# t-taniai/LocalExpStereo

Hardware: AMD Instinct MI355X
Metric: Mcost-evals/s (pixels x hypotheses / s), guided-filter cost aggregation, 1500x1000x256 vol (higher is better)
Workload: dtype i32 fixed-point box sums (exact; i64 stage-2 window sums), f32 3x3 algebra and combination

## Files before the change

### localexpstereo_amd/csrc/les_hip_march.inc

```
int check_rects(const les_hip_ctx* c, const les_hip_rect& f, const les_hip_rect& t)
{
    if (f.w < 0 || f.h < 0 || t.w < 0 || t.h < 0) return fail(LES_HIP_ERR_ARG, "negative rect size");
    if (f.x < 0 || f.y < 0 || f.x + f.w > c->p.W || f.y + f.h > c->p.H) return fail(LES_HIP_ERR_ARG, "filterRect outside the image");
    if (t.w > 0 && t.h > 0 && (t.x < f.x || t.y < f.y || t.x + t.w > f.x + f.w || t.y + t.h > f.y + f.h))
        return fail(LES_HIP_ERR_ARG, "targetRect not inside filterRect");
    return LES_HIP_OK;
}

int build_jobs(const les_hip_ctx* c, int n, const les_hip_rect* frs, const les_hip_rect* trs, int out_slabs,
               std::vector<les::Job>& jobs)
{
    const int TW = c->strip->TW, R = c->R;
    const long long P = (long long)c->p.H * c->p.W;
    long long strips = 0;
    for (int i = 0; i < n; i++) {
        int rc = check_rects(c, frs[i], trs[i]);
        if (rc) return rc;
        if (trs[i].w > 0 && trs[i].h > 0) strips += (trs[i].w + TW - 1) / TW;
    }
    int max_rows = 1 << 30;
    if (strips > 0 && strips < 2048) {
        long long want = (2048 + strips - 1) / strips;
        int tallest = 0;
        for (int i = 0; i < n; i++) tallest = std::max(tallest, trs[i].h);
        max_rows = std::max<long long>(std::max(8 * R, 64), (tallest + want - 1) / want);
    }
    jobs.clear();
    for (int i = 0; i < n; i++) {
        const les_hip_rect &f = frs[i], &t = trs[i];
        if (t.w <= 0 || t.h <= 0) continue;
        for (int sy = 0; sy < t.h; sy += max_rows)
            for (int sx = 0; sx < t.w; sx += TW) {
                les::Job j;
                j.tx0 = t.x + sx; j.ty0 = t.y + sy;
                j.tw = std::min(TW, t.w - sx); j.th = std::min(max_rows, t.h - sy);
                j.cx0 = f.x; j.cy0 = f.y; j.cx1 = f.x + f.w; j.cy1 = f.y + f.h;
                j.out_off = (out_slabs ? (long long)(i / out_slabs) * P : 0) + (long long)j.ty0 * c->p.W + j.tx0;
                j.out_stride = c->p.W;
                j.plane_idx = i;
                jobs.push_back(j);
            }
    }
    std::stable_sort(jobs.begin(), jobs.end(), [](const les::Job& a, const les::Job& b) {
        if (a.tx0 != b.tx0) return a.tx0 < b.tx0;
        if (a.ty0 != b.ty0) return a.ty0 < b.ty0;
        return a.plane_idx < b.plane_idx;
    });
    return LES_HIP_OK;
}

bool build_march_jobs(les_hip_ctx* c, int n, const les_hip_rect* frs, const les_hip_rect* trs, int out_slabs,
                      std::vector<les::Job>& jobs, bool& ok, const MarchEntry*& entry)
{
    jobs.clear();
    ok = false;
    entry = nullptr;
    if (!c->march) return true;
    const int R = c->R, W = c->p.W, H = c->p.H;
    const long long P = (long long)H * W;
    ok = true;
    for (int i = 0; i < n; i++) {
        const les_hip_rect &f = frs[i], &t = trs[i];
        if (t.w <= 0 || t.h <= 0) continue;
        if ((f.x > 0 && t.x - f.x < 2 * R) || (f.x + f.w < W && (f.x + f.w) - (t.x + t.w) < 2 * R) ||
            (f.y > 0 && t.y - f.y < 2 * R) || (f.y + f.h < H && (f.y + f.h) - (t.y + t.h) < 2 * R)) ok = false;
    }
    if (!ok) {
        note_fallback(c->fallback_seen, FB_GEOMETRY, "a target rectangle lies closer than 2 x radius = %d pixels to a filterRect border that is not an image border", 2 * R);
        return true;
    }
    const int ncu = c->ncu;
    const MarchEntry* cands[2] = {c->march, find_march(c->R, 0)};
    const MarchEntry* m = c->march;
    int max_rows = 1 << 30;
    {
        double best = 1e300;
        const int row_opts[] = {1 << 30, 1024, 512, 384, 256, 192, 128, 96, 64, 48, 32};
        for (int g = 0; g < 2; g++) {
            const MarchEntry* e = cands[g];
            if (!e || (g == 1 && e == cands[0])) continue;
            if (const char* w = getenv("LES_HIP_MARCH_WIDE")) if ((atoi(w) != 0) != (g == 0)) continue;
            for (int ro : row_opts) {
                long long njobs = 0;
                int rows = 0, useful = 0;
                for (int i = 0; i < n; i++) {
                    const les_hip_rect& t = trs[i];
                    if (t.w <= 0 || t.h <= 0) continue;
                    const int ns = (t.w + e->TW - 1) / e->TW;
                    const int nr = (t.h + ro - 1) / ro, sh = (t.h + nr - 1) / nr;
                    njobs += (long long)ns * nr;
                    rows = std::max(rows, sh);
                    useful = std::max(useful, (t.w + ns - 1) / ns);
                }
                if (njobs == 0) continue;
                const long long wgs = (njobs + e->NJ - 1) / e->NJ;
                const double ticks = (double)((rows + 4 * R + e->BY - 1) / e->BY + 3);
                const double cost = (double)((wgs + ncu - 1) / ncu) * ticks * (1.0 + 1e-3 * (double)wgs / ncu) + (ro == (1 << 30) ? 0.0 : 1e-6);
                if (cost < best) { best = cost; m = e; max_rows = ro; }
            }
        }
    }
    if (const char* e = getenv("LES_HIP_MARCH_ROWS")) max_rows = std::max(1, atoi(e));
    entry = m;
    const int TW = m->TW, NJ = m->NJ;
    for (int i = 0; i < n; i++) {
        const les_hip_rect &f = frs[i], &t = trs[i];
        if (t.w <= 0 || t.h <= 0) continue;
        const int ns = (t.w + TW - 1) / TW, sw = (t.w + ns - 1) / ns;
        const int nr = (t.h + max_rows - 1) / max_rows, sh = (t.h + nr - 1) / nr;
        for (int sy = 0; sy < t.h; sy += sh)
            for (int sx = 0; sx < t.w; sx += sw) {
                les::Job j;
                j.tx0 = t.x + sx; j.ty0 = t.y + sy;
                j.tw = std::min(sw, t.w - sx); j.th = std::min(sh, t.h - sy);
                j.cx0 = f.x; j.cy0 = f.y; j.cx1 = f.x + f.w; j.cy1 = f.y + f.h;
                j.out_off = (out_slabs ? (long long)(i / out_slabs) * P : 0) + (long long)j.ty0 * W + j.tx0;
                j.out_stride = W;
                j.plane_idx = i;
                jobs.push_back(j);
            }
    }
    std::stable_sort(jobs.begin(), jobs.end(), [](const les::Job& a, const les::Job& b) {
        if (a.tx0 != b.tx0) return a.tx0 < b.tx0;
        if (a.ty0 != b.ty0) return a.ty0 < b.ty0;
        return a.plane_idx < b.plane_idx;
    });
    while (!jobs.empty() && jobs.size() % NJ) {
        les::Job pad = jobs.back();
        pad.tw = 0; pad.th = 0;
        jobs.push_back(pad);
    }
    return true;
}

int ensure_planes(les_hip_ctx* c, size_t n)
{
    if (n <= c->planes_cap) return LES_HIP_OK;
    if (c->d_planes) HIPCHECK(hipFree(c->d_planes));
    c->d_planes = nullptr; c->planes_cap = 0;
    size_t cap = std::max<size_t>(n, 1024);
    HIPCHECK(hipMalloc((void**)&c->d_planes, cap * sizeof(float4)));
    c->planes_cap = cap;
    return LES_HIP_OK;
}

struct RawPatches { const les::RawCall* calls; const long long* off; float* raw; int n, chunks; };

les::View strip_view(const les_hip_ctx* c, int mode)
{
    les::View view{c->v[mode].vol, c->v[mode].stats, c->v[mode].ipk, c->v[mode].ipk10, nullptr, nullptr, mode ? -1.0f : 1.0f, c->th_color, c->th_grad};
    if (c->naive) { view.feat_self = c->v[mode].feat; view.feat_other = c->v[1 - mode].feat; }
    return view;
}

int launch_march(les_hip_ctx* c, const MarchEntry* m, int mode, const les::Job* d_mjobs, int ngroups, const float4* d_planes, float* d_out, int check,
                 hipStream_t stream, const RawPatches* rp = nullptr)
{
    if (ngroups <= 0) return LES_HIP_OK;
    les::MarchView mv = c->v[mode].mv;
    if (c->naive) {
        if (!rp || !rp->raw || !c->v[1 - mode].feat) return fail(LES_HIP_ERR_ARG, "view %d was not supplied at creation", mode);
        hipLaunchKernelGGL(les::les_naive_raw_kernel, dim3(rp->n, rp->chunks), dim3(256), 0, stream, c->geom, strip_view(c, mode), rp->calls, d_planes, rp->raw);
        mv.vol = rp->raw; mv.raw_off = rp->off;
    }
    hipLaunchKernelGGL(m->fn, dim3(ngroups), dim3(m->NT), 0, stream, c->geom, mv, d_mjobs, d_planes, d_out, ngroups, check);
    HIPCHECK(hipGetLastError());
    return LES_HIP_OK;
}

const StripEntry* strip_for(const les_hip_ctx* c) { return (c->naive || c->interp == 1) ? c->strip : c->istrip[c->interp == 0 ? 0 : 1]; }

int launch_strips(les_hip_ctx* c, int mode, const les::Job* d_jobs, int njobs, const float4* d_planes, float* d_out, int check, hipStream_t stream)
{
    if (njobs <= 0) return LES_HIP_OK;
    if (mode < 0 || mode > 1 || !c->v[mode].stats || (c->naive ? !c->v[1 - mode].feat : !c->v[mode].vol))
        return fail(LES_HIP_ERR_ARG, "view %d was not supplied at creation", mode);
    const StripEntry* se = strip_for(c);
    if (!se) return fail(LES_HIP_ERR_UNSUPPORTED, "no strip kernel for interpolation %d at guided-filter radius %d", c->interp, c->R);
    const les::View view = strip_view(c, mode);
    hipLaunchKernelGGL(se->fn, dim3(njobs), dim3(se->NT), 0, stream, c->geom, view, d_jobs, d_planes, d_out, njobs, check);
    HIPCHECK(hipGetLastError());
    return LES_HIP_OK;
}

bool interp_march_ok(const les_hip_ctx* c, int mode)
{
    return !c->naive && c->interp != 1 && c->march && c->v[mode].march_ok && (c->interp == 0 || c->v[mode].march2_ok);
}

int launch_nan_spread(les_hip_ctx* c, int mode, int n, const les::RawCall* calls, const les::WtaJob* targets, const long long* out_off, int stride,
                      const float4* d_planes, const unsigned* flags, float* d_out, int check, hipStream_t stream)
{
    if (n <= 0) return LES_HIP_OK;
    if (c->interp == 2)
        hipLaunchKernelGGL(les::les_nan_spread_kernel<2>, dim3(n), dim3(256), 0, stream, c->geom, (const float*)c->v[mode].vol, calls, targets, out_off, stride,
                           d_planes, flags, d_out, 2 * c->R, check);
    else
        hipLaunchKernelGGL(les::les_nan_spread_kernel<0>, dim3(n), dim3(256), 0, stream, c->geom, (const float*)c->v[mode].vol, calls, targets, out_off, stride,
                           d_planes, flags, d_out, 2 * c->R, check);
    HIPCHECK(hipGetLastError());
    return LES_HIP_OK;
}

int launch_interp_march(les_hip_ctx* c, const MarchEntry* m, int mode, const les::Job* d_mjobs, int ngroups, const RawPatches& rp,
                        unsigned* d_flags, const les::Job* d_sjobs, les::Job* d_rjobs, int nsjobs, const les::WtaJob* targets, const long long* out_off,
                        int stride, const float4* d_planes, float* d_out, int check, hipStream_t stream)
{
    const ViewData& v = c->v[mode];
    const bool quad = c->interp == 2;
    les::MarchView mv = quad ? v.mv2 : v.mv;
    mv.vol = rp.raw; mv.raw_off = rp.off; mv.vol_t = nullptr;
    if (quad) {
        if (!c->istrip[1]) return fail(LES_HIP_ERR_UNSUPPORTED, "no strip kernel for interpolation 2 at guided-filter radius %d", c->R);
        HIPCHECK(hipMemsetAsync(d_flags, 0, (size_t)rp.n * sizeof(unsigned), stream));
        hipLaunchKernelGGL(les::les_interp_raw_kernel<2>, dim3(rp.n, rp.chunks), dim3(256), 0, stream, c->geom, (const float*)v.vol, rp.calls, d_planes,
                           rp.raw, d_flags, v.lo2);
    } else {
        hipLaunchKernelGGL(les::les_interp_raw_kernel<0>, dim3(rp.n, rp.chunks), dim3(256), 0, stream, c->geom, (const float*)v.vol, rp.calls, d_planes,
                           rp.raw, (unsigned*)nullptr, -INFINITY);
    }
    HIPCHECK(hipGetLastError());
    if (ngroups > 0) hipLaunchKernelGGL(m->fn, dim3(ngroups), dim3(m->NT), 0, stream, c->geom, mv, d_mjobs, d_planes, d_out, ngroups, check);
    HIPCHECK(hipGetLastError());
    if (quad && nsjobs > 0) {
        hipLaunchKernelGGL(les::les_mask_jobs_kernel, dim3((nsjobs + 255) / 256), dim3(256), 0, stream, d_sjobs, d_rjobs, (const unsigned*)d_flags, nsjobs);
        HIPCHECK(hipGetLastError());
        const StripEntry* se = c->istrip[1];
        hipLaunchKernelGGL(se->fn, dim3(nsjobs), dim3(se->NT), 0, stream, c->geom, strip_view(c, mode), (const les::Job*)d_rjobs, d_planes, d_out, nsjobs, check);
        HIPCHECK(hipGetLastError());
        return launch_nan_spread(c, mode, rp.n, rp.calls, targets, out_off, stride, d_planes, d_flags, d_out, check, stream);
    }
    return LES_HIP_OK;
}

float naive_alpha(const les_hip_ctx* c);

int build_march_view(les_hip_ctx* c, int m, const double* d_hs)
{
    ViewData& v = c->v[m];
    const size_t P = (size_t)c->p.H * c->p.W;
    const int W = c->p.W, H = c->p.H;
    v.march_ok = false;
    v.march2_ok = false;
    if ((unsigned long long)P * (4ull * les::kMarchStatWords) >= (1ull << 31)) {
        note_fallback(c->fallback_seen, FB_IMAGE_SIZE, "image of %d x %d pixels (32-bit row offsets reach 2^26 pixels)", W, H);
        return LES_HIP_OK;
    }
    const float th = c->naive ? c->th_color + c->th_grad : c->p.th_col;
    if (!(th > 0.0f) || !(th < INFINITY)) { note_fallback(c->fallback_seen, FB_THRESHOLD, "truncation threshold %g is not positive and finite", (double)th); return LES_HIP_OK; }
    if (d_hs) {
        unsigned dbits = 0;
        struct DevBuf { void* p = nullptr; ~DevBuf() { if (p) (void)hipFree(p); } } dm;
        HIPCHECK(hipMalloc(&dm.p, sizeof(unsigned)));
        unsigned* d_dmax = static_cast<unsigned*>(dm.p);
        HIPCHECK(hipMemsetAsync(d_dmax, 0, sizeof(unsigned), cur_stream(c)));
        HIPCHECK(hipMalloc((void**)&v.ipk8, P * sizeof(uint32_t)));
        HIPCHECK(hipMalloc((void**)&v.mstats, P * les::kMarchStatWords * sizeof(float)));
        hipLaunchKernelGGL(les::les_march_stats_kernel, dim3((W + 255) / 256, H), dim3(256), 0, cur_stream(c), d_hs, v.ipk, v.ipk8, v.mstats, d_dmax, H, W, c->R, c->p.eps);
        HIPCHECK(hipGetLastError());
        HIPCHECK(hipMemcpyAsync(&dbits, d_dmax, sizeof(unsigned), hipMemcpyDeviceToHost, cur_stream(c)));
        HIPCHECK(hipStreamSynchronize(cur_stream(c)));
        v.dmax_bits = dbits;
    }
    auto drop_tiled = [&]() { if (v.vol_t) { (void)hipFree(v.vol_t); v.vol_t = nullptr; } };
    const int nb = 2048;
    std::vector<float> hmin(nb, 0.0f); std::vector<int> hbad(nb, 0);
    if (!c->naive) {
        struct DevBuf { void* p = nullptr; ~DevBuf() { if (p) (void)hipFree(p); } } part;
        HIPCHECK(hipMalloc(&part.p, nb * (sizeof(float) + sizeof(int))));
        float* d_min = static_cast<float*>(part.p);
        int* d_bad = reinterpret_cast<int*>(d_min + nb);
        hipLaunchKernelGGL(les::les_range_kernel, dim3(nb), dim3(256), 0, cur_stream(c), v.vol, P * (size_t)c->p.D, d_min, d_bad);
        HIPCHECK(hipGetLastError());
        HIPCHECK(hipMemcpyAsync(hmin.data(), d_min, nb * sizeof(float), hipMemcpyDeviceToHost, cur_stream(c)));
        HIPCHECK(hipMemcpyAsync(hbad.data(), d_bad, nb * sizeof(int), hipMemcpyDeviceToHost, cur_stream(c)));
        HIPCHECK(hipStreamSynchronize(cur_stream(c)));
    }
    float vmin = INFINITY; int bad = 0;
    for (int i = 0; i < nb; i++) { vmin = std::min(vmin, hmin[i]); bad |= hbad[i]; }
    if (bad || !(vmin < INFINITY)) {
        note_fallback(c->fallback_seen, FB_NONFINITE, "the cost volume of view %d holds NaN or infinite entries", m);
        drop_tiled();
        return LES_HIP_OK;
    }
    vmin = std::min(vmin, 0.5f * th);
    const double range = (double)th - (double)vmin;
    if (!(range <= 8.0 * (double)th)) {
        note_fallback(c->fallback_seen, FB_RANGE, "view %d: costs reach %g below the truncation threshold %g (more than 8 x the threshold)", m, range, (double)th);
        drop_tiled();
        return LES_HIP_OK;
    }
    const unsigned dbits = v.dmax_bits;
    float dmax;
    memcpy(&dmax, &dbits, sizeof dmax);
    if (!(dmax > 0.0f) || !(dmax < INFINITY)) { note_fallback(c->fallback_seen, FB_GUIDE, "view %d: the inverse covariance of the guide is not positive and finite (largest diagonal entry %g)", m, (double)dmax); return LES_HIP_OK; }
    const int K = 2 * c->R + 1;
    auto scaled_view = [&](float lo) {
        const double range = (double)th - (double)lo;
        const double Ba = 0.5 * range * std::sqrt((double)dmax), Bb = range + 1.5 * Ba;
        const double scale = 1073741824.0 / ((double)K * Bb * 1.25);
        const int PB = les::march_pb(c->R);
        const float spf = (float)((double)((1 << PB) - 1) / range);
        const double c0 = std::rint(-(double)lo * (double)spf) - (double)(1 << (PB - 1));
        const double up = 1.0 / (double)spf;
        les::MarchView mv;
        mv.vol = v.vol; mv.ipk8 = v.ipk8; mv.mstats = v.mstats;
        mv.sp = spf;
        mv.pmagic = (float)(12582912.0 + c0);
        mv.poff = (float)(-c0 * up);
        mv.kapS = (float)((double)(1 << les::kMarchSH) * up / 255.0 * scale);
        mv.upS = (float)(up * scale);
        mv.qscale = (float)((double)(1 << les::kMarchS2) / (255.0 * scale));
        mv.kmu = (float)(1.0 / ((double)(1ll << les::kMarchMB) * 255.0));
        mv.raw_off = nullptr;
        mv.vol_t = nullptr;
        return mv;
    };
    les::MarchView mv = scaled_view(vmin);
    if (!c->naive) {
        const float lo2 = (float)((double)vmin - 0.5 * range);
        if ((double)th - (double)lo2 <= 8.0 * (double)th) {
            v.mv2 = scaled_view(lo2);
            v.lo2 = lo2;
            v.march2_ok = true;
        }
    }
    if (!c->naive && v.vol) {
        const char* e = getenv("LES_HIP_TILED");
        const unsigned long long nt = (unsigned long long)H * (unsigned long long)((W + 7) / 8) * 8ull * (unsigned long long)c->p.D;
        if (!(e && atoi(e) == 0) && (unsigned long long)((W + 7) / 8) * (unsigned long long)c->p.D * 32ull < (1ull << 31)) {
            if (v.vol_t) { (void)hipFree(v.vol_t); v.vol_t = nullptr; }
            size_t mem_free = 0, mem_total = 0;
            const bool room = hipMemGetInfo(&mem_free, &mem_total) == hipSuccess && mem_free >= 2 * nt * sizeof(float) + (4ull << 30);
            if (room && hipMalloc((void**)&v.vol_t, nt * sizeof(float)) == hipSuccess) {
                hipLaunchKernelGGL(les::les_tile_volume_kernel, dim3((unsigned)(((W + 7) / 8 * 8 + 63) / 64), (unsigned)H), dim3(256), 0, cur_stream(c), v.vol, v.vol_t, c->p.D, H, W);
                HIPCHECK(hipGetLastError());
                mv.vol_t = v.vol_t;
            } else {
                (void)hipGetLastError();
                v.vol_t = nullptr;
            }
        }
    }
    v.mv = mv;
    v.march_ok = true;
    return LES_HIP_OK;
}

int build_view(les_hip_ctx* c, int m, const uint8_t* im, const float* vol)
{
    const size_t P = (size_t)c->p.H * c->p.W;
    ViewData& v = c->v[m];
    if (vol) {
        if (c->p.volumes_on_device) { v.vol = const_cast<float*>(vol); v.own_vol = false; }
        else {
            HIPCHECK(hipMalloc((void**)&v.vol, P * c->p.D * sizeof(float)));
            v.own_vol = true;
            HIPCHECK(hipMemcpy(v.vol, vol, P * c->p.D * sizeof(float), hipMemcpyHostToDevice));
        }
    }
    if (!im) return LES_HIP_OK;
    uint8_t* d_img = nullptr;
    double* d_hs = nullptr;
    HIPCHECK(hipMalloc((void**)&d_img, P * 3));
    HIPCHECK(hipMemcpy(d_img, im, P * 3, hipMemcpyHostToDevice));
    HIPCHECK(hipMalloc((void**)&v.ipk, P * sizeof(uint32_t)));
    HIPCHECK(hipMalloc((void**)&v.ipk10, P * sizeof(uint32_t)));
    HIPCHECK(hipMalloc((void**)&v.stats, (P * 3 + 1) * sizeof(float4)));
    HIPCHECK(hipMemsetAsync(v.stats + P * 3, 0, sizeof(float4), cur_stream(c)));
    HIPCHECK(hipMalloc((void**)&d_hs, P * 9 * sizeof(double)));
    const int W = c->p.W, H = c->p.H;
    if (c->naive) {
        HIPCHECK(hipMalloc((void**)&v.feat, P * sizeof(float4)));
        hipLaunchKernelGGL(les::les_naive_features_kernel, dim3((c->p.W + 255) / 256, c->p.H), dim3(256), 0, cur_stream(c), d_img, v.feat, c->p.H, c->p.W, naive_alpha(c));
    }
    hipLaunchKernelGGL(les::les_pack_guide_kernel, dim3((unsigned)((P + 255) / 256)), dim3(256), 0, cur_stream(c), d_img, v.ipk, v.ipk10, (int)P);
    hipLaunchKernelGGL(les::les_stats_hsum_kernel, dim3((W + 255) / 256, H), dim3(256), 0, cur_stream(c), v.ipk, d_hs, H, W, c->R);
    hipLaunchKernelGGL(les::les_stats_finish_kernel, dim3((W + 255) / 256, H), dim3(256), 0, cur_stream(c), d_hs, v.stats, H, W, c->R, c->p.eps);
    HIPCHECK(hipGetLastError());
    if (c->march && (v.vol || c->naive)) {
        int rc = build_march_view(c, m, d_hs);
        if (rc) { (void)hipFree(d_img); (void)hipFree(d_hs); return rc; }
    }
    HIPCHECK(hipStreamSynchronize(cur_stream(c)));
    HIPCHECK(hipFree(d_img));
    HIPCHECK(hipFree(d_hs));
    return LES_HIP_OK;
}
```

### localexpstereo_amd/csrc/les_hip_march_tables.inc

```
typedef void (*StripKernel)(les::Geom, les::View, const les::Job*, const float4*, float*, int, int);
struct StripEntry { int R; int variant; int TW; int NT; StripKernel fn; };

#define LES_STRIP_ENTRY(R_, V_, WA_, BY_, SEG_, MW_) \
    { R_, V_, les::StripCfg<R_, WA_, BY_, SEG_>::TW, les::StripCfg<R_, WA_, BY_, SEG_>::NT, les::les_strip_kernel<R_, WA_, BY_, SEG_, MW_> }
const StripEntry kStrips[] = {
    LES_STRIP_ENTRY(1, 0, 64, 16, 4, 2), LES_STRIP_ENTRY(2, 0, 64, 16, 4, 2), LES_STRIP_ENTRY(3, 0, 64, 16, 4, 2),
    LES_STRIP_ENTRY(4, 0, 64, 16, 4, 2), LES_STRIP_ENTRY(5, 0, 64, 16, 4, 2), LES_STRIP_ENTRY(6, 0, 64, 16, 4, 2),
    LES_STRIP_ENTRY(7, 0, 64, 16, 4, 2), LES_STRIP_ENTRY(8, 0, 64, 16, 4, 2), LES_STRIP_ENTRY(9, 0, 64, 16, 4, 2),
    LES_STRIP_ENTRY(10, 0, 64, 21, 3, 3), LES_STRIP_ENTRY(12, 0, 64, 16, 4, 2), LES_STRIP_ENTRY(15, 0, 96, 16, 6, 2),
    LES_STRIP_ENTRY(10, 8, 128, 21, 6, 2), LES_STRIP_ENTRY(10, 11, 64, 21, 3, 2),
};
#define LES_NAIVE_ENTRY(R_, WA_, BY_, SEG_, MW_) \
    { R_, 0, les::StripCfg<R_, WA_, BY_, SEG_>::TW, les::StripCfg<R_, WA_, BY_, SEG_>::NT, les::les_strip_kernel<R_, WA_, BY_, SEG_, MW_, 1> }
const StripEntry kNaiveStrips[] = {
    LES_NAIVE_ENTRY(1, 64, 16, 4, 2), LES_NAIVE_ENTRY(2, 64, 16, 4, 2), LES_NAIVE_ENTRY(3, 64, 16, 4, 2), LES_NAIVE_ENTRY(4, 64, 16, 4, 2),
    LES_NAIVE_ENTRY(5, 64, 16, 4, 2), LES_NAIVE_ENTRY(6, 64, 16, 4, 2), LES_NAIVE_ENTRY(7, 64, 16, 4, 2), LES_NAIVE_ENTRY(8, 64, 16, 4, 2),
    LES_NAIVE_ENTRY(9, 64, 16, 4, 2), LES_NAIVE_ENTRY(10, 64, 16, 4, 2), LES_NAIVE_ENTRY(12, 64, 16, 4, 2), LES_NAIVE_ENTRY(15, 96, 16, 6, 2),
};
#define LES_INTERP_ENTRY(R_, WA_, BY_, SEG_, MW_, SRC_) \
    { R_, 0, les::StripCfg<R_, WA_, BY_, SEG_>::TW, les::StripCfg<R_, WA_, BY_, SEG_>::NT, les::les_strip_kernel<R_, WA_, BY_, SEG_, MW_, SRC_> }
#define LES_INTERP_ENTRIES(SRC_) \
    LES_INTERP_ENTRY(1, 64, 16, 4, 2, SRC_), LES_INTERP_ENTRY(2, 64, 16, 4, 2, SRC_), LES_INTERP_ENTRY(3, 64, 16, 4, 2, SRC_), \
    LES_INTERP_ENTRY(4, 64, 16, 4, 2, SRC_), LES_INTERP_ENTRY(5, 64, 16, 4, 2, SRC_), LES_INTERP_ENTRY(6, 64, 16, 4, 2, SRC_), \
    LES_INTERP_ENTRY(7, 64, 16, 4, 2, SRC_), LES_INTERP_ENTRY(8, 64, 16, 4, 2, SRC_), LES_INTERP_ENTRY(9, 64, 16, 4, 2, SRC_), \
    LES_INTERP_ENTRY(10, 64, 16, 4, 2, SRC_), LES_INTERP_ENTRY(12, 64, 16, 4, 2, SRC_), LES_INTERP_ENTRY(15, 96, 16, 6, 2, SRC_)
const StripEntry kNearestStrips[] = { LES_INTERP_ENTRIES(2) };
const StripEntry kQuadraticStrips[] = { LES_INTERP_ENTRIES(3) };
const StripEntry* find_interp_strip(int R, int interp)
{
    for (const auto& e : (interp == 0 ? kNearestStrips : kQuadraticStrips))
        if (e.R == R) return &e;
    return nullptr;
}
const StripEntry* find_naive_strip(int R)
{
    for (const auto& e : kNaiveStrips)
        if (e.R == R) return &e;
    return nullptr;
}
const StripEntry* find_strip(int R)
{
    int variant = 0;
    if (const char* v = getenv("LES_HIP_VARIANT")) variant = atoi(v);
    const StripEntry* def = nullptr;
    for (const auto& e : kStrips) {
        if (e.R != R) continue;
        if (e.variant == variant) return &e;
        if (e.variant == 0) def = &e;
    }
    return def;
}

typedef void (*MarchKernel)(les::Geom, les::MarchView, const les::Job*, const float4*, float*, int, int);
struct MarchEntry { int R; int TW; int NJ; int NT; int BY; MarchKernel fn; };
#define LES_MARCH_ENTRY(R_, WGC_, NJ_, BY_) \
    { R_, les::MarchCfg<R_, WGC_, NJ_, BY_>::TW, NJ_, les::MarchCfg<R_, WGC_, NJ_, BY_>::NT, BY_, les::les_march_kernel<R_, WGC_, NJ_, BY_> }
const MarchEntry kMarch[] = {
    LES_MARCH_ENTRY(10, 256, 1, 7),
#if defined(LES_MARCH_LAB) && defined(LES_MARCH_NARROW_NJ1)
    LES_MARCH_ENTRY(10, 128, 1, 7),
#else
    LES_MARCH_ENTRY(10, 128, 2, 7),
#endif
    LES_MARCH_ENTRY(7, 256, 1, 5),
    LES_MARCH_ENTRY(7, 128, 2, 5),
#if !defined(LES_MARCH_FEW_RADII)
    LES_MARCH_ENTRY(2, 256, 1, 2),  LES_MARCH_ENTRY(2, 128, 2, 2),
    LES_MARCH_ENTRY(3, 256, 1, 3),  LES_MARCH_ENTRY(3, 128, 2, 3),
    LES_MARCH_ENTRY(4, 256, 1, 3),  LES_MARCH_ENTRY(4, 128, 2, 3),
    LES_MARCH_ENTRY(5, 256, 1, 4),  LES_MARCH_ENTRY(5, 128, 2, 4),
    LES_MARCH_ENTRY(6, 256, 1, 5),  LES_MARCH_ENTRY(6, 128, 2, 5),
    LES_MARCH_ENTRY(8, 256, 1, 6),  LES_MARCH_ENTRY(8, 128, 2, 6),
    LES_MARCH_ENTRY(9, 256, 1, 7),  LES_MARCH_ENTRY(9, 128, 2, 7),
#endif
};
const MarchEntry* find_march(int R, int wide = 1)
{
    if (const char* k = getenv("LES_HIP_KERNEL")) if (!strcmp(k, "strip")) return nullptr;
    const MarchEntry* best = nullptr;
    for (const auto& e : kMarch)
        if (e.R == R && (!best || (wide ? e.TW > best->TW : e.TW < best->TW))) best = &e;
    return best;
}

constexpr long long kRawPatchCapFloats = 1ll << 30;
constexpr int kRansacMaxSam = 500;
constexpr int kRansacChunks = 5;
constexpr int kRansacChunkEnds[kRansacChunks] = {16, 64, 128, 256, kRansacMaxSam};
```

### localexpstereo_amd/csrc/les_hip_vdisp.inc

```

void launch_naive_raw(les_hip_ctx* c, int mode, const les::RawCall* calls, int n, int chunks, const float4* d_planes, float* raw, hipStream_t stream)
{
    hipLaunchKernelGGL(les::les_naive_raw_v_kernel, dim3(n, chunks), dim3(256), 0, stream, c->geom, strip_view(c, mode), calls, d_planes, raw, 0, 0,
                       (unsigned*)nullptr);
}

int launch_naive_march(les_hip_ctx* c, const MarchEntry* m, int mode, const les::Job* d_mjobs, int ngroups, const float4* d_planes, float* d_out, int check,
                       hipStream_t stream, const RawPatches& rp)
{
    if (ngroups <= 0) return LES_HIP_OK;
    if (!rp.raw || !c->v[1 - mode].feat) return fail(LES_HIP_ERR_ARG, "view %d was not supplied at creation", mode);
    launch_naive_raw(c, mode, rp.calls, rp.n, rp.chunks, d_planes, rp.raw, stream);
    les::MarchView mv = c->v[mode].mv;
    mv.vol = rp.raw; mv.raw_off = rp.off;
    hipLaunchKernelGGL(m->fn, dim3(ngroups), dim3(m->NT), 0, stream, c->geom, mv, d_mjobs, d_planes, d_out, ngroups, check);
    HIPCHECK(hipGetLastError());
    return LES_HIP_OK;
}

constexpr long long kVdispVolCapFloats = 1ll << 28;

void vdisp_layout(const les_hip_ctx* c, int n, const les_hip_rect* frs, const les_hip_rect* trs, UnaryTables& t, std::vector<les::RawCall>& calls,
                  std::vector<float4>& stand)
{
    const long long HW = (long long)c->p.H * c->p.W;
    const int cap = (int)std::max<long long>(1, kVdispVolCapFloats / std::max<long long>(HW, 1));
    calls.resize((size_t)n);
    stand.resize((size_t)n);
    std::vector<std::vector<les_hip_rect>> used;
    VdispGroup g{0, 0, 0};
    long long amax = 1;
    for (int i = 0; i < n; i++) {
        const les_hip_rect f = frs[i];
        const bool live = trs[i].w > 0 && trs[i].h > 0 && f.w > 0 && f.h > 0;
        int s = 0;
        if (live) {
            auto overlaps = [&](const les_hip_rect& r) { return f.x < r.x + r.w && r.x < f.x + f.w && f.y < r.y + r.h && r.y < f.y + f.h; };
            for (s = 0; s < (int)used.size(); s++) {
                bool free_ = true;
                for (const auto& r : used[s]) if (overlaps(r)) { free_ = false; break; }
                if (free_) break;
            }
            if (s == (int)used.size()) {
                if (s == cap) {
                    g.c1 = i; g.slices = s; t.vd_groups.push_back(g);
                    g = VdispGroup{i, i, 0};
                    used.clear(); s = 0;
                }
                used.emplace_back();
            }
            used[s].push_back(f);
            amax = std::max(amax, (long long)f.w * f.h);
        }
        calls[i] = les::RawCall{f.x, f.y, live ? f.w : 0, live ? f.h : 0, (long long)s * HW + (long long)f.y * c->p.W + f.x};
        stand[i] = make_float4(0.0f, 0.0f, (float)s, 0.0f);
    }
    g.c1 = n; g.slices = (int)used.size(); t.vd_groups.push_back(g);
    for (const auto& gg : t.vd_groups) t.vd_max_slices = std::max(t.vd_max_slices, gg.slices);
    t.vd_chunks = (int)std::min<long long>(1024, std::max<long long>(1, (amax + 4095) / 4096));
}

int launch_vdisp_strips(les_hip_ctx* c, const UnaryTables& t, float* vol, unsigned* flags, les::Job* rjobs, int mode, const float4* d_planes,
                        float* d_out, int check, hipStream_t stream)
{
    const int njobs = t.njobs;
    if (njobs <= 0 || t.n <= 0 || t.vd_max_slices <= 0) return LES_HIP_OK;
    const StripEntry* se = find_interp_strip(c->R, 0);
    if (!se || se->TW < c->strip->TW)
        return fail(LES_HIP_ERR_UNSUPPORTED, "no nearest-slice strip kernel for guided-filter radius %d (vertical disparity on the strip path)", c->R);
    les::Geom g = c->geom;
    g.D0 = 0; g.th_col = INFINITY;
    les::View view = strip_view(c, mode);
    view.vol = vol;
    const les::RawCall* vd_calls = t.d_vd_calls;
    const les::Job* jobs = t.d_jobs;
    const float4* stand_in = t.d_vd_stand_in;
    for (const auto& gr : t.vd_groups) {
        if (gr.c1 <= gr.c0 || gr.slices <= 0) continue;
        g.D = gr.slices;
        if (t.vd_groups.size() > 1) HIPCHECK(hipMemsetAsync(flags, 0, (size_t)t.n * sizeof(unsigned), stream));
        hipLaunchKernelGGL(les::les_naive_raw_v_kernel, dim3(gr.c1 - gr.c0, t.vd_chunks), dim3(256), 0, stream, c->geom, strip_view(c, mode),
                           vd_calls + gr.c0, d_planes + gr.c0, vol, c->p.W, 1, flags + gr.c0);
        hipLaunchKernelGGL(les::les_mask_jobs_kernel, dim3((njobs + 255) / 256), dim3(256), 0, stream, jobs, rjobs, (const unsigned*)flags, njobs);
        hipLaunchKernelGGL(se->fn, dim3(njobs), dim3(se->NT), 0, stream, g, view, (const les::Job*)rjobs, stand_in, d_out, njobs, 0);
        if (check)
            hipLaunchKernelGGL(les::les_vdisp_check_kernel, dim3(njobs), dim3(256), 0, stream, c->geom, (const les::Job*)rjobs, d_planes, d_out, njobs);
        HIPCHECK(hipGetLastError());
    }
    return LES_HIP_OK;
}
```

### localexpstereo_amd/csrc/les_march.h

```cpp
#pragma once

#include "les_kernels.h"

#if defined(LES_MARCH_LAB)
#include "les_march_lab.h"
#else
#define LES_MARCH_ROLE_ORDER 5
#define LES_STATS_POLICY ""
#define LES_LAB_ROLE_ON(bit) true
#define LES_LAB_ABLATE(bit) false
#endif
#ifndef LES_TICK_BEGIN
#define LES_TICK_BEGIN() ((void)0)
#define LES_TICK_MARK() ((void)0)
#define LES_TICK_BARRIER() __syncthreads()
#define LES_TICK_END(role_) ((void)0)
#endif

namespace les {

constexpr int kMarchSH = 5;
constexpr int kMarchMB = 24;
constexpr int kMarchSL = 3;
constexpr int kMarchS2 = 4;
constexpr int kMarchMagicBits = 0x4B400000;
static_assert(kMarchSH + kMarchMB + kMarchSL == 32, "N cov = t - hi32(M * (s << SL)) needs the scales to meet at 2^32");
__host__ __device__ constexpr int march_pb(int R) { return (2 * R + 1) * (2 * R + 1) < 512 ? 20 : 19; }
#ifndef LES_MARCH_STAT_WORDS
#define LES_MARCH_STAT_WORDS 9
#endif
constexpr int kMarchStatWords = LES_MARCH_STAT_WORDS;
static_assert(kMarchStatWords == 9 || kMarchStatWords == 12, "statistics record of 36 or 48 bytes");

struct MarchView {
    const float* vol;
    const uint32_t* ipk8;
    const float* mstats;
    float sp;
    float pmagic;
    float poff;
    float kapS;
    float upS;
    float qscale;
    float kmu;
    const long long* raw_off;
    const float* vol_t;
};
#ifndef LES_TILED_MIN_SLOPE_WIDE
#define LES_TILED_MIN_SLOPE_WIDE 0.05f
#endif
#ifndef LES_TILED_MIN_SLOPE
#define LES_TILED_MIN_SLOPE 0.125f
#endif

template <int R, int WGC, int NJ, int BY>
struct MarchCfg {
    static constexpr int KS = 2 * R + 1;
    static constexpr int RS = 3 * BY;
    static constexpr int TW = WGC - 4 * R;
    static constexpr int HWV = WGC / 64;
    static constexpr int NW = 3 * HWV * NJ;
    static constexpr int NT = 64 * NW;
    static constexpr int SEGL = 8;
    static constexpr int PADW = 16;
    static constexpr int PCOLS0 = 1 + WGC + WGC / PADW;
    static constexpr int PCOLS = PCOLS0 + ((4 - PCOLS0 % 8) + 8) % 8;
    static_assert(RS >= KS, "the ring must hold a whole window (the row that leaves it is the one written KS rows ago)");
    static_assert(RS - KS < BY, "a ring longer than the window by a block or more wastes registers: pick the smallest block height");
    static_assert(WGC % 64 == 0, "a job slot is a whole number of waves");
    static_assert(BY * (64 / SEGL) <= 64, "one wave prefixes its own tile");
    static_assert(TW > 0, "job too narrow for this radius");
    static_assert(2 * R + 1 < 64, "a window crosses at most one wave boundary");
    static_assert((long long)KS * KS * (1ll << (march_pb(R) - 1 + kMarchSL)) < (1ll << 31), "stage-1 window sums (shifted for the product with M) must fit int32");
    static_assert((long long)KS * 128 * (1ll << (march_pb(R) - 1)) < (1ll << 31), "vertical sums of Iq * pi must fit int32");
    static_assert((long long)KS * (1ll << (30 - kMarchS2)) < (1ll << 31), "the stage-2 window sums, rounded to 2^S2, must fit int32");
    __host__ __device__ static constexpr int pcol(int ci) { return 1 + ci + ci / PADW; }
};

__device__ __forceinline__ void march_prefix_scan8(int4 (&v)[8])
{
#pragma unroll
    for (int j = 1; j < 8; j++) { v[j].x += v[j - 1].x; v[j].y += v[j - 1].y; v[j].z += v[j - 1].z; v[j].w += v[j - 1].w; }
    int4 inc = v[7];
#if defined(LES_SIM) || defined(LES_MARCH_SCAN_PLAIN)
#define LES_SCAN_STEP(N) { inc.x += dpp_row_shr<N>(inc.x); inc.y += dpp_row_shr<N>(inc.y); inc.z += dpp_row_shr<N>(inc.z); inc.w += dpp_row_shr<N>(inc.w); }
    LES_SCAN_STEP(2) LES_SCAN_STEP(4) LES_SCAN_STEP(8)
#undef LES_SCAN_STEP
#else
#define LES_SCAN_ROW(N) "v_add_u32_dpp %0, %0, %0 row_shr:" #N " row_mask:0xf bank_mask:0xf bound_ctrl:1\n" \
                        "v_add_u32_dpp %1, %1, %1 row_shr:" #N " row_mask:0xf bank_mask:0xf bound_ctrl:1\n" \
                        "v_add_u32_dpp %2, %2, %2 row_shr:" #N " row_mask:0xf bank_mask:0xf bound_ctrl:1\n" \
                        "v_add_u32_dpp %3, %3, %3 row_shr:" #N " row_mask:0xf bank_mask:0xf bound_ctrl:1\n"
    asm("s_nop 1\n" LES_SCAN_ROW(2) LES_SCAN_ROW(4) LES_SCAN_ROW(8) : "+v"(inc.x), "+v"(inc.y), "+v"(inc.z), "+v"(inc.w));
#undef LES_SCAN_ROW
#endif
    const int4 off = int4{inc.x - v[7].x, inc.y - v[7].y, inc.z - v[7].z, inc.w - v[7].w};
#pragma unroll
    for (int j = 0; j < 8; j++) { v[j].x += off.x; v[j].y += off.y; v[j].z += off.z; v[j].w += off.w; }
}

template <int BY, int PCOLS>
__device__ __forceinline__ void march_prefix_tile(int4 (*T)[PCOLS], int ci0, int lane)
{
    constexpr int SEGL = 8;
    const int row = 2 * (lane >> 4) + (lane & 1), seg = (lane & 15) >> 1;
    const bool act = row < BY;
    const int c0 = ci0 + seg * SEGL;
    int4* p = &T[act ? row : 0][1 + c0 + c0 / 16];
    int4 v[SEGL];
#pragma unroll
    for (int j = 0; j < SEGL; j++) v[j] = p[j];
    march_prefix_scan8(v);
    if (act) {
#pragma unroll
        for (int j = 0; j < SEGL; j++) lds_store4(&p[j], v[j].x, v[j].y, v[j].z, v[j].w);
    }
}

template <int BY, int PCOLS>
__device__ __forceinline__ void march_prefix_pair(int4 (*TA)[PCOLS], int4 (*TB)[PCOLS], int ci0, int lane)
{
    constexpr int SEGL = 8;
    const int row = 2 * (lane >> 4) + (lane & 1), seg = (lane & 15) >> 1;
    const bool act = row < BY;
    const int c0 = ci0 + seg * SEGL;
    const int pc = 1 + c0 + c0 / 16;
    int4* pa = &TA[act ? row : 0][pc];
    int4* pb = &TB[act ? row : 0][pc];
    int4 va[SEGL], vb[SEGL];
#pragma unroll
    for (int j = 0; j < SEGL; j++) vb[j] = pb[j];
    wave_sync();
#pragma unroll
    for (int j = 0; j < SEGL; j++) va[j] = pa[j];
    LES_MARCH_SCHED_FENCE();
    march_prefix_scan8(vb);
    if (act) {
#pragma unroll
        for (int j = 0; j < SEGL; j++) lds_store4(&pb[j], vb[j].x, vb[j].y, vb[j].z, vb[j].w);
    }
    LES_MARCH_SCHED_FENCE();
    march_prefix_scan8(va);
    if (act) {
#pragma unroll
        for (int j = 0; j < SEGL; j++) lds_store4(&pa[j], va[j].x, va[j].y, va[j].z, va[j].w);
    }
}

#if defined(LES_SIM)
typedef float4 mstat4;
#else
typedef float mstat4 __attribute__((ext_vector_type(4)));
#endif
#if LES_MARCH_STAT_WORDS == 9
typedef float mstat_tail;
#else
typedef mstat4 mstat_tail;
#endif
struct MarchStatRow { mstat4 a, b; mstat_tail c; };
#if defined(LES_SIM) || defined(LES_MARCH_STATS_PLAIN)
struct MarchStatDesc { const char* base; uint32_t bytes; };
__device__ inline MarchStatDesc march_stats_desc(const float* base, uint32_t bytes) { return MarchStatDesc{(const char*)base, bytes}; }
__device__ inline void march_stats_load(MarchStatRow& r, const MarchStatDesc& d, uint32_t voff, uint32_t soff)
{
    const unsigned long long o = (unsigned long long)voff + (unsigned long long)soff;
    float w[8 + sizeof(mstat_tail) / 4];
    for (unsigned i = 0; i < sizeof w / 4; i++) w[i] = (o + 4ull * i + 4 <= d.bytes) ? *reinterpret_cast<const float*>(d.base + o + 4ull * i) : 0.0f;
    memcpy(&r.a, w, 16); memcpy(&r.b, w + 4, 16); memcpy(&r.c, w + 8, sizeof r.c);
}
template <int N>
__device__ inline void march_stats_wait(MarchStatRow& r) { (void)r; }
template <int N>
__device__ inline void march_stats_wait(MarchStatRow& r, MarchStatRow& q) { (void)r; (void)q; }
#else
typedef int MarchStatDesc __attribute__((ext_vector_type(4)));
__device__ __forceinline__ MarchStatDesc march_stats_desc(const float* base, uint32_t bytes)
{
    const unsigned long long a = (unsigned long long)base;
    MarchStatDesc d;
    d.x = __builtin_amdgcn_readfirstlane((int)(uint32_t)a);
    d.y = __builtin_amdgcn_readfirstlane((int)((uint32_t)(a >> 32) & 0xffffu));
    d.z = __builtin_amdgcn_readfirstlane((int)bytes);
    d.w = 0x00027000;
    return d;
}
__device__ __forceinline__ void march_stats_load(MarchStatRow& r, const MarchStatDesc& d, uint32_t voff, uint32_t soff)
{
    asm volatile("buffer_load_dwordx4 %0, %1, %2, %3 offen" LES_STATS_POLICY : "+v"(r.a) : "v"(voff), "s"(d), "s"(soff));
    asm volatile("buffer_load_dwordx4 %0, %1, %2, %3 offen offset:16" LES_STATS_POLICY : "+v"(r.b) : "v"(voff), "s"(d), "s"(soff));
#if LES_MARCH_STAT_WORDS == 9
    asm volatile("buffer_load_dword %0, %1, %2, %3 offen offset:32" LES_STATS_POLICY : "+v"(r.c) : "v"(voff), "s"(d), "s"(soff));
#else
    asm volatile("buffer_load_dwordx4 %0, %1, %2, %3 offen offset:32" LES_STATS_POLICY : "+v"(r.c) : "v"(voff), "s"(d), "s"(soff));
#endif
}
template <int N>
__device__ __forceinline__ void march_stats_wait(MarchStatRow& r) { asm volatile("s_waitcnt vmcnt(%3)" : "+v"(r.a), "+v"(r.b), "+v"(r.c) : "n"(N)); }
template <int N>
__device__ __forceinline__ void march_stats_wait(MarchStatRow& r, MarchStatRow& q)
{
    asm volatile("s_waitcnt vmcnt(%6)" : "+v"(r.a), "+v"(r.b), "+v"(r.c), "+v"(q.a), "+v"(q.b), "+v"(q.c) : "n"(N));
}
#endif
__device__ __forceinline__ int march_stat_m2(const MarchStatRow& r)
{
#if LES_MARCH_STAT_WORDS == 9
    return __float_as_int(r.c);
#else
    return __float_as_int(r.c.x);
#endif
}

__device__ __forceinline__ bool march_label_surely_valid(const Geom& g, float4 pl, int x0, int x1, int y0, int y1)
{
    const float ax0 = pl.x * (float)x0, ax1 = pl.x * (float)x1, by0 = pl.y * (float)y0, by1 = pl.y * (float)y1;
    const float spread = 5.0f * (fabsf(pl.x) + fabsf(pl.y));
    const float lo = (fminf(ax0, ax1) + fminf(by0, by1)) + pl.z - spread;
    const float hi = (fmaxf(ax0, ax1) + fmaxf(by0, by1)) + pl.z + spread;
    const float mag = fmaxf(fabsf(ax0), fabsf(ax1)) + fmaxf(fabsf(by0), fabsf(by1)) + fabsf(pl.z) + spread;
    const float margin = 1e-5f * mag + 1e-30f;
    return (0.0f * pl.w == 0.0f) && mag < 1e30f && (lo - margin >= g.mind) && (hi + margin <= g.maxd);
}

__device__ __forceinline__ bool march_plane_short_gather(const Geom& g, float4 pl, const Job& job, int R, int* slice_lo)
{
    *slice_lo = 0;
    const unsigned long long HW = (unsigned long long)g.H * (unsigned long long)g.W;
    const bool moderate = fabsf(pl.x) < 1e30f && fabsf(pl.y) < 1e30f && fabsf(pl.z) < 1e30f;
    if (!(moderate && g.mind == 0.0f && g.D0 == 0 && g.maxd == (float)(g.D - 1) && g.D >= 2 && HW < (1ull << 24))) return false;
    if ((unsigned long long)g.D * HW < (1ull << 30)) return true;
    const int x0 = max(job.tx0 - 2 * R, job.cx0), x1 = min(job.tx0 + job.tw + 2 * R, job.cx1) - 1;
    const int y0 = max(job.ty0 - 2 * R, job.cy0), y1 = min(job.ty0 + job.th + 2 * R, job.cy1) - 1;
    if (x1 < x0 || y1 < y0) return false;
    const float ax0 = pl.x * (float)x0, ax1 = pl.x * (float)x1, by0 = pl.y * (float)y0, by1 = pl.y * (float)y1;
    const float lo = (fminf(ax0, ax1) + fminf(by0, by1)) + pl.z, hi = (fmaxf(ax0, ax1) + fmaxf(by0, by1)) + pl.z;
    const float mag = fmaxf(fabsf(ax0), fabsf(ax1)) + fmaxf(fabsf(by0), fabsf(by1)) + fabsf(pl.z);
    const float margin = 1e-5f * mag + 1e-30f;
    if (!((lo - margin >= 0.0f) && (hi + margin < g.maxd))) return false;
    const int s0 = (int)floorf(lo - margin), s1 = (int)floorf(hi + margin) + 1;
    *slice_lo = s0;
    return s0 >= 0 && s1 < g.D && (unsigned long long)(s1 - s0 + 1) * HW < (1ull << 28);
}

template <int R, int WGC, int NJ, int BY>
__global__ void __launch_bounds__(3 * WGC * NJ)
les_march_kernel(Geom g, MarchView view, const Job* __restrict__ jobs, const float4* __restrict__ planes,
                 float* __restrict__ out, int ngroups, int check)
{
    using Cfg = MarchCfg<R, WGC, NJ, BY>;
    constexpr int KS = Cfg::KS, RS = Cfg::RS, NT = Cfg::NT, HWV = Cfg::HWV, PCOLS = Cfg::PCOLS;
    constexpr int UN = 3;

    __shared__ int4 s_T1[2][NJ][BY][PCOLS];
    __shared__ int4 s_T2[3][NJ][BY][PCOLS];
    __shared__ float s_rtab[KS + 1];

    int grp;
    {
        const int nwg = (int)gridDim.x, orig = (int)blockIdx.x;
        const int q = nwg / 8, r = nwg % 8, xcd = orig % 8;
        grp = (xcd < r ? xcd * (q + 1) : r * (q + 1) + (xcd - r) * q) + orig / 8;
    }
    if (grp >= ngroups) return;
    const int tid = (int)threadIdx.x;
    const int lane = tid & 63;
    const int wave = readfirstlane_i32(tid >> 6);
    constexpr int kRoleOf[6][3] = {{0, 1, 2}, {2, 1, 0}, {1, 2, 0}, {2, 0, 1}, {1, 0, 2}, {0, 2, 1}};
    const int slot = wave / (3 * HWV), role = kRoleOf[LES_MARCH_ROLE_ORDER][(wave % (3 * HWV)) / HWV], half = wave % HWV;
    const int ci0 = half * 64, ci = ci0 + lane;
    const Job job = jobs[grp * NJ + slot];
    int th_max = 0;
#pragma unroll
    for (int s = 0; s < NJ; s++) th_max = max(th_max, jobs[grp * NJ + s].th);
    const int nblk = (th_max + 4 * R + BY - 1) / BY;
    const int nticks = nblk + 3;
    const int Ttot = job.th > 0 ? job.th + 4 * R : 0;
    const float4 plane = planes[job.plane_idx];
    const int cy1m = max(job.cy1 - 1, job.cy0);

    if (tid <= KS) s_rtab[tid] = tid > 0 ? (float)(1.0 / (double)tid) : 0.0f;
    for (int k = tid; k < 3 * NJ * BY; k += NT) {
        if (k < 2 * NJ * BY) (&s_T1[0][0][0][0])[k * PCOLS] = int4{0, 0, 0, 0};
        (&s_T2[0][0][0][0])[k * PCOLS] = int4{0, 0, 0, 0};
    }
    __syncthreads();

    const int gx = job.tx0 - 2 * R + ci;
    const bool col_in = gx >= job.cx0 && gx < job.cx1 && job.th > 0;
    const int sx = min(max(gx, job.cx0), max(job.cx1 - 1, job.cx0));
    const uint32_t sx4 = (uint32_t)sx * 4u;
    const uint32_t rowB = (uint32_t)g.W * 4u;
    const uint32_t imgB = (uint32_t)g.H * rowB;
    const BufRsrc rs_guide = make_buf(view.ipk8, imgB);
    const int nx = window_count(gx, R, job.cx0, job.cx1);
    const int cP = min(ci + R, WGC - 1), cM = ci - R - 1;
    const int pcP = Cfg::pcol(cP);
    const int pcM = cM >= 0 ? Cfg::pcol(cM) : 0;
    const bool cross = cM >= 0 && (cP >> 6) != (cM >> 6);
    const int pcX = cross ? Cfg::pcol((cP >> 6) * 64 - 1) : 0;
    const int pcS = Cfg::pcol(ci);

    if (role == 0 && LES_LAB_ROLE_ON(1)) {
        const uint32_t HWu = (uint32_t)g.H * (uint32_t)g.W;
        const float g_ax = plane.x * (float)sx;
        const bool fronto = plane.x == 0.0f && plane.y == 0.0f;
        GatherPrep gpc = gather_prepare(g, 0.0f, plane.z, 0u, HWu, true);
        if (gpc.f1 == 0.0f) gpc.i1 = gpc.i0;
        int ringN[RS];
        uint32_t ringG[RS];
#pragma unroll
        for (int k = 0; k < RS; k++) { ringN[k] = 0; ringG[k] = 0u; }
        int Sp = 0;
        int Sc[3] = {1 << (kMarchSH - 1), 1 << (kMarchSH - 1), 1 << (kMarchSH - 1)};
        const uint32_t i0s = (uint32_t)readfirstlane_i32((int)gpc.i0), i1s = (uint32_t)readfirstlane_i32((int)gpc.i1);
        const float f1s = __int_as_float(readfirstlane_i32(__float_as_int(gpc.f1)));
        const int modes = readfirstlane_i32(gpc.mode);
        const float f0s = 1.0f - f1s;
        const bool inv_job = fronto && modes == 2 && !view.raw_off;
        int slice_lo = 0;
        const bool tame = !fronto && !view.raw_off && march_plane_short_gather(g, plane, job, R, &slice_lo);
        const uint32_t W8 = ((uint32_t)g.W + 7u) >> 3;
        const uint32_t trowB = W8 * (uint32_t)g.D * 32u;
        const int trow_lo = max(job.ty0 - 2 * R, job.cy0);
        const int trow_hi = min(job.ty0 - 2 * R + (nblk + 2) * BY, job.cy1);
        const unsigned long long tspanB = (unsigned long long)max(trow_hi - trow_lo, 1) * (unsigned long long)trowB;
        const bool tiled = tame && view.vol_t && fabsf(plane.x) >= (NJ == 1 ? LES_TILED_MIN_SLOPE_WIDE : LES_TILED_MIN_SLOPE) && tspanB < 0xfffffff0ull &&
                           (unsigned long long)W8 * (unsigned long long)g.D * 32ull < (1ull << 31);
        const float spj = !col_in ? 0.0f : (inv_job ? 0.0f : view.sp);
        const float pmj = !col_in ? __int_as_float(kMarchMagicBits) : (inv_job ? fmaf(g.th_col, view.sp, view.pmagic) : view.pmagic);
        auto march_a = [&](auto kind_tag) __attribute__((always_inline)) {
        constexpr int KIND = decltype(kind_tag)::value;
        GatherPrep gp[BY];
        float v0[BY], v1[BY];
        float f1r[BY];
        uint32_t gw[BY];
        uint32_t rowbits = 0, rowbits_nx = 0;
        int nx_rowB = 0;
        float nx_dbase = 0.0f;
        int nx_rowraw = 0;
        int nx_rowT = 0;
        const int fw = job.cx1 - job.cx0;
        const float* v0base = view.vol + (size_t)i0s;
        if constexpr (KIND == 3) v0base = view.vol + view.raw_off[job.plane_idx] - job.cx0;
        if constexpr (KIND == 4) v0base = view.vol + (size_t)slice_lo * (size_t)HWu;
        if constexpr (KIND == 5) v0base = view.vol_t + (size_t)trow_lo * (size_t)(trowB >> 2);
        const unsigned long long rest4 = (unsigned long long)(g.D - slice_lo) * (unsigned long long)imgB;
        const unsigned long long trestB = (unsigned long long)(g.H - trow_lo) * (unsigned long long)trowB;
        const uint32_t tiledB = (uint32_t)(trestB < 0xfffffffcull ? trestB : 0xfffffffcull);
        const BufRsrc rs_v0 = make_buf(v0base, KIND == 3 ? 0xfffffffcu : (KIND == 4 ? (uint32_t)(rest4 < 0xfffffffcull ? rest4 : 0xfffffffcull) : (KIND == 5 ? tiledB : imgB)));
        const uint32_t tcol = (((uint32_t)sx >> 3) * (uint32_t)g.D * 8u + ((uint32_t)sx & 7u)) * 4u;
        const int dsub = g.D0 - slice_lo;
        const BufRsrc rs_v1 = make_buf(view.vol + (size_t)i1s, imgB);
        auto prep = [&](int b) __attribute__((always_inline)) {
            const int t = b * BY + lane;
            const int gy = job.ty0 - 2 * R + t;
            const int sy = min(max(gy, job.cy0), cy1m);
            nx_rowB = (int)((uint32_t)sy * rowB);
            rowbits_nx = ballot_low(t < Ttot && gy >= job.cy0 && gy < job.cy1, BY);
            if constexpr (KIND == 3) nx_rowraw = (sy - job.cy0) * fw * 4;
            else nx_dbase = plane.y * (float)sy + plane.z;
            if constexpr (KIND == 5) nx_rowT = (int)((uint32_t)(sy - trow_lo) * trowB);
        };
        auto issue_row = [&](auto itag) __attribute__((always_inline)) {
            constexpr int i = decltype(itag)::value;
            const uint32_t ro = (uint32_t)readlane_i32(nx_rowB, i);
            if (LES_LAB_ABLATE(64)) { v0[i] = (float)lane; v1[i] = 0.0f; gw[i] = (uint32_t)lane; return; }
            if constexpr (KIND == 3) {
                v0[i] = buf_load<float>(rs_v0, sx4, (uint32_t)readlane_i32(nx_rowraw, i));
            } else if constexpr (KIND < 2) {
                v0[i] = buf_load<float>(rs_v0, sx4, ro);
                if constexpr (KIND == 1) v1[i] = buf_load<float>(rs_v1, sx4, ro);
            } else if constexpr (KIND == 4) {
                const float d = g_ax + readlane_f32(nx_dbase, i);
                const float dc = med3_f32(d, 0.0f, g.maxd);
                const float df = floorf(dc);
                f1r[i] = dc - df;
                const uint32_t e = mad_u24((int)df + dsub, (int)HWu, sx);
                v0[i] = buf_load<float>(rs_v0, e << 2, ro);
                v1[i] = buf_load<float>(rs_v0, (e << 2) + (f1r[i] > 0.0f ? imgB : 0u), ro);
            } else if constexpr (KIND == 5) {
                const float d = g_ax + readlane_f32(nx_dbase, i);
                const float dc = med3_f32(d, 0.0f, g.maxd);
                const float df = floorf(dc);
                f1r[i] = dc - df;
                const uint32_t e = (((uint32_t)(int)df + (uint32_t)g.D0) << 5) + tcol;
                const uint32_t rt = (uint32_t)readlane_i32(nx_rowT, i);
                v0[i] = buf_load<float>(rs_v0, e, rt);
                v1[i] = buf_load<float>(rs_v0, e + (f1r[i] > 0.0f ? 32u : 0u), rt);
            } else {
                const float d_base = readlane_f32(nx_dbase, i);
                const bool inside = col_in && ((rowbits_nx >> i) & 1u);
                gp[i] = gather_prepare(g, g_ax, d_base, (ro >> 2) + (uint32_t)sx, HWu, inside);
                if (gp[i].f1 == 0.0f) gp[i].i1 = gp[i].i0;
                v0[i] = view.vol[gp[i].i0];
                v1[i] = view.vol[gp[i].i1];
            }
            gw[i] = buf_load<uint32_t>(rs_guide, sx4, ro);
        };
        prep(0);
        rowbits = rowbits_nx;
        prep(0);
        static_for<BY>([&](auto itag) { issue_row(itag); });
        LES_TICK_BEGIN();
        for (int k0 = 0; k0 < nticks; k0 += UN) {
            static_for<UN>([&](auto utag) {
                constexpr int BASE = decltype(utag)::value * BY;
                const int k = k0 + decltype(utag)::value;
                if (k < nticks) {
                    if (k < nblk) {
                        int4 (*T)[PCOLS] = s_T1[k & 1][slot];
                        prep(k + 1);
                        static_for<BY>([&](auto itag) {
                            constexpr int i = decltype(itag)::value;
                            constexpr int SLOT = BASE + i;
                            constexpr int OLD = (SLOT + RS - KS) % RS;
                            int pi;
                            if constexpr (KIND == 3) {
                                pi = (__float_as_int(fmaf(v0[i], spj, pmj)) - kMarchMagicBits) & sbfe1(rowbits, i);
                            } else if constexpr (KIND < 2) {
                                float C = v0[i];
                                if constexpr (KIND == 1) C = f0s * v0[i] + f1s * v1[i];
                                const float p = min_f32_finite(C, g.th_col);
                                pi = (__float_as_int(fmaf(p, spj, pmj)) - kMarchMagicBits) & sbfe1(rowbits, i);
                            } else if constexpr (KIND == 4 || KIND == 5) {
                                const float f0 = 1.0f - f1r[i];
                                const float C = f0 * v0[i] + f1r[i] * v1[i];
                                const float p = min_f32_finite(C, g.th_col);
                                pi = (__float_as_int(fmaf(p, spj, pmj)) - kMarchMagicBits) & sbfe1(rowbits, i);
                            } else {
                                const float p = gather_finish(g, gp[i], v0[i], v1[i]);
                                pi = __float_as_int(fmaf(p, view.sp, view.pmagic)) - kMarchMagicBits;
                                pi = gp[i].mode == 3 ? 0 : pi;
                            }
                            const uint32_t gi = gw[i];
                            const int no = ringN[OLD];
                            const uint32_t go = ringG[OLD];
                            ringN[SLOT] = -pi;
                            ringG[SLOT] = gi;
                            Sp = Sp + pi + no;
                            Sc[0] = Sc[0] + mul24_sbyte<0>(gi, pi) + mul24_sbyte<0>(go, no);
                            Sc[1] = Sc[1] + mul24_sbyte<1>(gi, pi) + mul24_sbyte<1>(go, no);
                            Sc[2] = Sc[2] + mul24_sbyte<2>(gi, pi) + mul24_sbyte<2>(go, no);
                            lds_store4(&T[i][pcS], Sp, Sc[0] >> kMarchSH, Sc[1] >> kMarchSH, Sc[2] >> kMarchSH);
                            issue_row(itag);
                        });
                        rowbits = rowbits_nx;
                        LES_TICK_MARK();
                    }
                    {
                        int4 (*TB)[PCOLS] = s_T2[(decltype(utag)::value + UN - 2 % UN) % UN][slot];
                        const bool da = k < nblk, db = !(NJ > 1 && KIND == 2) && k >= 2 && k < nblk + 2;
                        constexpr bool kPair = KIND != 2 && KIND != 4 && KIND != 5;
                        if (kPair && da && db) march_prefix_pair<BY, PCOLS>(s_T1[k & 1][slot], TB, ci0, lane);
                        else {
                            if (da) { wave_sync(); march_prefix_tile<BY, PCOLS>(s_T1[k & 1][slot], ci0, lane); }
                            if (db) march_prefix_tile<BY, PCOLS>(TB, ci0, lane);
                        }
                    }
                    LES_TICK_BARRIER();
                }
            });
        }
        LES_TICK_END(0);
        };
        if (view.raw_off) march_a(std::integral_constant<int, 3>{});
        else if (fronto && f1s == 0.0f) march_a(std::integral_constant<int, 0>{});
        else if (fronto) march_a(std::integral_constant<int, 1>{});
        else if (tiled) march_a(std::integral_constant<int, 5>{});
        else if (tame) march_a(std::integral_constant<int, 4>{});
        else march_a(std::integral_constant<int, 2>{});
    } else if (role == 1 && LES_LAB_ROLE_ON(2)) {
        const bool s1_col = col_in && ci >= R && ci < WGC - R;
        int slice_lo_unused = 0;
        const bool general_plane = !view.raw_off && !(plane.x == 0.0f && plane.y == 0.0f) && !march_plane_short_gather(g, plane, job, R, &slice_lo_unused);
        const float kap_x = s1_col ? view.kapS * s_rtab[nx] : 0.0f;
        const float up_x = s1_col ? view.upS * s_rtab[nx] : 0.0f;
        const uint32_t sxS = (uint32_t)sx * (uint32_t)(4 * kMarchStatWords);
        const uint32_t rowS = (uint32_t)g.W * (uint32_t)(4 * kMarchStatWords);
        const MarchStatDesc ds_stats = march_stats_desc(view.mstats, (uint32_t)g.H * rowS);
        MarchStatRow st[BY];
#pragma unroll
        for (int i = 0; i < BY; i++) {
            st[i].a = st[i].b = mstat4{0.0f, 0.0f, 0.0f, 0.0f};
#if LES_MARCH_STAT_WORDS == 9
            st[i].c = 0.0f;
#else
            st[i].c = mstat4{0.0f, 0.0f, 0.0f, 0.0f};
#endif
        }
        float rny[BY];
        int nx_srow = 0;
        float nx_rny = 0.0f;
        auto prep = [&](int b) __attribute__((always_inline)) {
            const int t = b * BY + lane;
            const int gy1 = job.ty0 - 3 * R + t;
            const bool on = gy1 >= job.cy0 && gy1 < job.cy1 && t >= 2 * R && t < Ttot;
            nx_rny = on ? s_rtab[window_count(gy1, R, job.cy0, job.cy1)] : 0.0f;
            nx_srow = (int)((uint32_t)min(max(gy1, job.cy0), cy1m) * rowS);
        };
        auto issue_row = [&](auto itag) __attribute__((always_inline)) {
            constexpr int i = decltype(itag)::value;
            rny[i] = readlane_f32(nx_rny, i);
            uint32_t soff = (uint32_t)readlane_i32(nx_srow, i) & 0xfffffffcu;
            if (LES_LAB_ABLATE(4)) soff &= 0x3u;
            if (LES_LAB_ABLATE(1)) return;
            march_stats_load(st[i], ds_stats, sxS, soff);
        };
        prep(0);
        static_for<BY>([&](auto itag) { issue_row(itag); });
        LES_TICK_BEGIN();
        for (int k = 0; k < nticks; k++) {
            if (k >= 1 && k <= nblk) {
                const int b = k - 1;
                const int4 (*T1)[PCOLS] = s_T1[b & 1][slot];
                int4 (*T2)[PCOLS] = s_T2[b % 3][slot];
                constexpr int GC = 2, NS = (BY + GC - 1) / GC;
                prep(k);
                int4 pp[2][GC], pm[2][GC], px[2][GC];
                auto lds_stage = [&](auto stag) __attribute__((always_inline)) {
                    constexpr int S = decltype(stag)::value;
#pragma unroll
                    for (int j = 0; j < GC; j++)
                        if (S * GC + j < BY) {
                            if (LES_LAB_ABLATE(2)) { pp[S & 1][j] = int4{lane, k, 2, 3}; pm[S & 1][j] = int4{3, 2, k, lane}; px[S & 1][j] = int4{0, 0, 0, 0}; }
                            else { pp[S & 1][j] = T1[S * GC + j][pcP]; pm[S & 1][j] = T1[S * GC + j][pcM]; px[S & 1][j] = T1[S * GC + j][pcX]; }
                        }
                };
                lds_stage(std::integral_constant<int, 0>{});
                static_for<NS>([&](auto gtag) {
                    constexpr int S = decltype(gtag)::value, CB = S & 1;
                    constexpr int LO = S * GC;
                    constexpr int N = (BY - LO) < GC ? (BY - LO) : GC;
                    if constexpr (S + 1 < NS) lds_stage(std::integral_constant<int, S + 1>{});
                    LES_MARCH_SCHED_FENCE();
                    static_assert(GC == 2, "vmcnt bookkeeping below is written for stages of two rows");
                    if constexpr (N == 2) march_stats_wait<3 * (BY - 2)>(st[LO], st[LO + 1]);
                    else march_stats_wait<3 * (BY - 1)>(st[LO]);
                    static_for<N>([&](auto jtag) {
                        constexpr int j = decltype(jtag)::value;
                        constexpr int i = LO + j;
                        const int s = pp[CB][j].x - pm[CB][j].x + px[CB][j].x;
                        const mstat4 q0 = st[i].a, q1 = st[i].b;
                        const int M0 = __float_as_int(q1.z), M1 = __float_as_int(q1.w), M2 = march_stat_m2(st[i]);
                        const long long s8 = (long long)(s << kMarchSL);
                        const float d0 = (float)((pp[CB][j].y - pm[CB][j].y) + px[CB][j].y + (int)(((long long)M0 * s8 + (1ll << 31)) >> 32));
                        const float d1 = (float)((pp[CB][j].z - pm[CB][j].z) + px[CB][j].z + (int)(((long long)M1 * s8 + (1ll << 31)) >> 32));
                        const float d2 = (float)((pp[CB][j].w - pm[CB][j].w) + px[CB][j].w + (int)(((long long)M2 * s8 + (1ll << 31)) >> 32));
                        const float ka = kap_x * rny[i];
                        const float a0 = fmaf(q0.z, d2, fmaf(q0.y, d1, q0.x * d0)) * ka;
                        const float a1 = fmaf(q1.x, d2, fmaf(q0.w, d1, q0.y * d0)) * ka;
                        const float a2 = fmaf(q1.y, d2, fmaf(q1.x, d1, q0.z * d0)) * ka;
                        const float mp = (float)s * (up_x * rny[i]);
#if LES_MARCH_STAT_WORDS == 9
                        const float bb = fmaf(view.kmu, fmaf(a2, (float)M2, fmaf(a1, (float)M1, a0 * (float)M0)), mp);
#else
                        const float bb = fmaf(-a2, st[i].c.w, fmaf(-a1, st[i].c.z, fmaf(-a0, st[i].c.y, mp)));
#endif
                        lds_store4(&T2[i][pcS], cvt_rpi_i32(a0), cvt_rpi_i32(a1), cvt_rpi_i32(a2), cvt_rpi_i32(bb));
                    });
                    LES_MARCH_SCHED_FENCE();
                    static_for<N>([&](auto jtag) { issue_row(std::integral_constant<int, LO + decltype(jtag)::value>{}); });
                });
                LES_TICK_MARK();
            }
            if (NJ > 1 && general_plane && k >= 2 && k < nblk + 2) march_prefix_tile<BY, PCOLS>(s_T2[(k - 2) % 3][slot], ci0, lane);
            LES_TICK_BARRIER();
        }
        LES_TICK_END(1);
    } else if (role == 2 && LES_LAB_ROLE_ON(4)) {
        const bool out_col = ci >= 2 * R && ci < 2 * R + job.tw && job.th > 0;
        const uint32_t oc4 = (uint32_t)max(ci - 2 * R, 0) * 4u;
        const float vl_xa = (float)gx * plane.x, vl_c = 1.0f * plane.z, vl_zv = 0.0f * plane.w, vl_a5 = plane.x * 5, vl_b5 = plane.y * 5;
        const float c_lane = view.qscale * s_rtab[nx];
        int ring2[4][RS];
#pragma unroll
        for (int k = 0; k < RS; k++) ring2[0][k] = ring2[1][k] = ring2[2][k] = ring2[3][k] = 0;
        long long S2[4] = {1ll << (kMarchS2 - 1), 1ll << (kMarchS2 - 1), 1ll << (kMarchS2 - 1), 1ll << (kMarchS2 - 1)};
        uint32_t gq[BY];
        float rny2[BY];
        uint32_t okbits = 0;
        int nx_grow = 0;
        float nx_rny = 0.0f;
        const BufRsrc rs_out = make_buf(out + job.out_off, 0xfffffffcu);
        const uint32_t ostrideB = (uint32_t)job.out_stride * 4u;
        auto prep = [&](int b) __attribute__((always_inline)) {
            const int t = b * BY + lane;
            const int gy2 = job.ty0 - 4 * R + t;
            nx_rny = s_rtab[window_count(gy2, R, job.cy0, job.cy1)];
            nx_grow = (int)((uint32_t)min(max(gy2, job.cy0), cy1m) * rowB);
            okbits = ballot_low(t >= 4 * R && t < Ttot, BY);
        };
        auto issue_row = [&](auto itag) __attribute__((always_inline)) {
            constexpr int i = decltype(itag)::value;
            rny2[i] = readlane_f32(nx_rny, i);
            if (LES_LAB_ABLATE(128)) { gq[i] = (uint32_t)lane; return; }
            gq[i] = buf_load<uint32_t>(rs_guide, sx4, (uint32_t)readlane_i32(nx_grow, i));
        };
        auto march_d = [&](auto check_tag) __attribute__((always_inline)) {
        constexpr bool CHECK = decltype(check_tag)::value != 0;
        LES_TICK_BEGIN();
        for (int k0 = 0; k0 < nticks; k0 += UN) {
            static_for<UN>([&](auto utag) {
                constexpr int U = decltype(utag)::value;
                constexpr int BASE = ((U + UN - 3 % UN) % UN) * BY;
                const int k = k0 + U;
                if (k < nticks) {
                    if (k >= 3) {
                        const int b = k - 3;
                        const int4 (*T2)[PCOLS] = s_T2[(U + UN - 3 % UN) % UN][slot];
                        constexpr int GD = 1, NS = (BY + GD - 1) / GD;
                        int4 pp[2][GD], pm[2][GD], px[2][GD];
                        auto lds_stage = [&](auto stag) __attribute__((always_inline)) {
                            constexpr int S = decltype(stag)::value;
#pragma unroll
                            for (int j = 0; j < GD; j++)
                                if (S * GD + j < BY) {
                                    if (LES_LAB_ABLATE(16)) { pp[S & 1][j] = int4{lane, b, 2, 3}; pm[S & 1][j] = int4{3, 2, b, lane}; px[S & 1][j] = int4{0, 0, 0, 0}; }
                                    else { pp[S & 1][j] = T2[S * GD + j][pcP]; pm[S & 1][j] = T2[S * GD + j][pcM]; px[S & 1][j] = T2[S * GD + j][pcX]; }
                                }
                        };
                        lds_stage(std::integral_constant<int, 0>{});
                        static_for<NS>([&](auto gtag) {
                            constexpr int S = decltype(gtag)::value, CB = S & 1;
                            constexpr int LO = S * GD;
                            constexpr int N = (BY - LO) < GD ? (BY - LO) : GD;
                            if constexpr (S + 1 < NS) lds_stage(std::integral_constant<int, S + 1>{});
                            LES_MARCH_SCHED_FENCE();
                            static_for<N>([&](auto jtag) {
                                constexpr int j = decltype(jtag)::value;
                                constexpr int i = LO + j;
                                constexpr int SLOT = BASE + i, OLD = (SLOT + RS - KS) % RS;
                                const int h0 = pp[CB][j].x - pm[CB][j].x + px[CB][j].x, h1 = pp[CB][j].y - pm[CB][j].y + px[CB][j].y;
                                const int h2 = pp[CB][j].z - pm[CB][j].z + px[CB][j].z, h3 = pp[CB][j].w - pm[CB][j].w + px[CB][j].w;
                                const int o0 = ring2[0][OLD], o1 = ring2[1][OLD], o2 = ring2[2][OLD], o3 = ring2[3][OLD];
                                ring2[0][SLOT] = h0; ring2[1][SLOT] = h1; ring2[2][SLOT] = h2; ring2[3][SLOT] = h3;
                                acc64_add_i32(S2[0], h0 - o0); acc64_add_i32(S2[1], h1 - o1); acc64_add_i32(S2[2], h2 - o2); acc64_add_i32(S2[3], h3 - o3);
                                if (out_col && ((okbits >> i) & 1u)) {
                                    const int t = b * BY + i;
                                    const uint32_t gi = gq[i];
                                    const float f0 = (float)(int)(S2[0] >> kMarchS2), f1 = (float)(int)(S2[1] >> kMarchS2), f2 = (float)(int)(S2[2] >> kMarchS2), f3 = (float)(int)(S2[3] >> kMarchS2);
                                    const float acc = fmaf(f2, cvt_f32_sbyte<2>(gi), fmaf(f1, cvt_f32_sbyte<1>(gi), fmaf(f0, cvt_f32_sbyte<0>(gi), f3 * 255.0f)));
                                    float q = fmaf(acc * c_lane, rny2[i], view.poff);
                                    if constexpr (CHECK) {
                                        const int gy2 = job.ty0 + t - 4 * R;
                                        const float ds = ((vl_xa + (float)gy2 * plane.y) + vl_c) + vl_zv;
                                        const float dp = ds + vl_a5, dm = ds - vl_a5;
                                        const float d1 = dp + vl_b5, d2 = dp - vl_b5, d3 = dm + vl_b5, d4 = dm - vl_b5;
                                        const float mn = fmin3(fmin3(ds, d1, d2), d3, d4), mx = fmax3(fmax3(ds, d1, d2), d3, d4);
                                        if (!(mn >= g.mind && mx <= g.maxd)) q = LES_COST_INVALID;
                                    }
                                    if (!(LES_LAB_ABLATE(128) && q != 12345.0f))
                                    buf_store<float>(rs_out, oc4, (uint32_t)(t - 4 * R) * ostrideB, q);
                                }
                            });
                            LES_MARCH_SCHED_FENCE();
                        });
                    }
                    if (k >= 2 && k <= nblk + 1) {
                        prep(k - 2);
                        static_for<BY>([&](auto itag) { issue_row(itag); });
                    }
                    LES_TICK_BARRIER();
                }
            });
        }
        LES_TICK_END(2);
        };
        const bool surely_valid = march_label_surely_valid(g, plane, job.tx0, job.tx0 + max(job.tw, 1) - 1, job.ty0, job.ty0 + max(job.th, 1) - 1);
        if (check && !surely_valid) march_d(std::integral_constant<int, 1>{});
        else march_d(std::integral_constant<int, 0>{});
    }
}

__global__ void les_march_stats_kernel(const double* __restrict__ hs, const uint32_t* __restrict__ ipk, uint32_t* __restrict__ ipk8,
                                       float* __restrict__ mstats, unsigned* __restrict__ inv_diag_max, int H, int W, int R, double eps)
{
    int x = (int)(blockIdx.x * blockDim.x + threadIdx.x), y = (int)blockIdx.y;
    if (x >= W) return;
    size_t P = (size_t)H * W;
    double s[9] = {0, 0, 0, 0, 0, 0, 0, 0, 0};
    for (int dy = -R; dy <= R; dy++) {
        int yy = y + dy;
        if (yy < 0 || yy >= H) continue;
        for (int k = 0; k < 9; k++) s[k] += hs[k * P + (size_t)yy * W + x];
    }
    double N = (double)(window_count(x, R, 0, W) * window_count(y, R, 0, H));
    double m0 = s[0] / N, m1 = s[1] / N, m2 = s[2] / N;
    double rr = s[3] / N - m0 * m0 + eps, rg = s[4] / N - m0 * m1, rb = s[5] / N - m0 * m2;
    double gg = s[6] / N - m1 * m1 + eps, gb = s[7] / N - m1 * m2, bb = s[8] / N - m2 * m2 + eps;
    double irr = gg * bb - gb * gb, irg = gb * rb - rg * bb, irb = rg * gb - gg * rb;
    double igg = rr * bb - rb * rb, igb = rb * rg - rr * gb, ibb = rr * gg - rg * rg;
    double det = irr * rr + irg * rg + irb * rb;
    irr /= det; irg /= det; irb /= det; igg /= det; igb /= det; ibb /= det;
    size_t px = (size_t)y * W + x;
    const double fs = (double)(1ll << kMarchMB);
    const double c0 = m0 * 255.0 - 128.0, c1 = m1 * 255.0 - 128.0, c2 = m2 * 255.0 - 128.0;
    const int M0 = (int)fmin(fmax(rint(-c0 * fs), -2147483648.0), 2147483647.0);
    const int M1 = (int)fmin(fmax(rint(-c1 * fs), -2147483648.0), 2147483647.0);
    const int M2 = (int)fmin(fmax(rint(-c2 * fs), -2147483648.0), 2147483647.0);
    float* o = mstats + px * kMarchStatWords;
    o[0] = (float)irr; o[1] = (float)irg; o[2] = (float)irb; o[3] = (float)igg;
    o[4] = (float)igb; o[5] = (float)ibb; o[6] = __int_as_float(M0); o[7] = __int_as_float(M1);
    o[8] = __int_as_float(M2);
    if (kMarchStatWords == 12) { o[9] = (float)(c0 / 255.0); o[10] = (float)(c1 / 255.0); o[11] = (float)(c2 / 255.0); }
    const uint32_t v = ipk[px];
    const uint32_t b0 = ((v & 0xffu) - 128u) & 0xffu, b1 = (((v >> 8) & 0xffu) - 128u) & 0xffu, b2 = (((v >> 16) & 0xffu) - 128u) & 0xffu;
    ipk8[px] = b0 | (b1 << 8) | (b2 << 16);
    const float dmax = fmaxf(fmaxf((float)irr, (float)igg), (float)ibb);
    if (dmax > 0.0f) atomicMax(inv_diag_max, __float_as_uint(dmax));
}

__global__ void les_tile_volume_kernel(const float* __restrict__ src, float* __restrict__ dst, int D, int H, int W)
{
    const int x = (int)(blockIdx.x * 64 + (threadIdx.x & 63)), y = (int)blockIdx.y;
    const int W8 = (W + 7) >> 3;
    if (x >= W8 * 8) return;
    const size_t HW = (size_t)H * W;
    float* o = dst + (((size_t)y * W8 + (size_t)(x >> 3)) * D) * 8 + (x & 7);
    for (int d = (int)(threadIdx.x >> 6); d < D; d += (int)(blockDim.x >> 6))
        o[(size_t)d * 8] = x < W ? src[(size_t)d * HW + (size_t)y * W + x] : 0.0f;
}

__global__ void les_range_kernel(const float* __restrict__ v, size_t n, float* __restrict__ part_min, int* __restrict__ part_bad)
{
    __shared__ float s_min[256];
    __shared__ int s_bad[256];
    float m = INFINITY;
    int bad = 0;
    for (size_t i = (size_t)blockIdx.x * blockDim.x + threadIdx.x; i < n; i += (size_t)gridDim.x * blockDim.x) {
        const float x = v[i];
        if (!(fabsf(x) < INFINITY)) bad = 1;
        else m = fminf(m, x);
    }
    s_min[threadIdx.x] = m; s_bad[threadIdx.x] = bad;
    __syncthreads();
    for (int k = 128; k > 0; k >>= 1) {
        if ((int)threadIdx.x < k) {
            s_min[threadIdx.x] = fminf(s_min[threadIdx.x], s_min[threadIdx.x + k]);
            s_bad[threadIdx.x] |= s_bad[threadIdx.x + k];
        }
        __syncthreads();
    }
    if (threadIdx.x == 0) { part_min[blockIdx.x] = s_min[0]; part_bad[blockIdx.x] = s_bad[0]; }
}

}
```

Baseline: 168,700.

## Skip out-of-image lead-in rows and lend stage-C rows to role A

```diff
diff --git a/localexpstereo_amd/csrc/les_hip_march.inc b/localexpstereo_amd/csrc/les_hip_march.inc
--- a/localexpstereo_amd/csrc/les_hip_march.inc
+++ b/localexpstereo_amd/csrc/les_hip_march.inc
@@ -49,6 +49,12 @@
     return LES_HIP_OK;
 }
 
+int march_sched()
+{
+    const char* e = getenv("LES_HIP_MARCH_SCHED");
+    return e ? atoi(e) & 3 : 3;
+}
+
 bool build_march_jobs(les_hip_ctx* c, int n, const les_hip_rect* frs, const les_hip_rect* trs, int out_slabs,
                       std::vector<les::Job>& jobs, bool& ok, const MarchEntry*& entry)
 {
@@ -69,7 +75,7 @@
         note_fallback(c->fallback_seen, FB_GEOMETRY, "a target rectangle lies closer than 2 x radius = %d pixels to a filterRect border that is not an image border", 2 * R);
         return true;
     }
-    const int ncu = c->ncu;
+    const int ncu = c->ncu, sched = march_sched();
     const MarchEntry* cands[2] = {c->march, find_march(c->R, 0)};
     const MarchEntry* m = c->march;
     int max_rows = 1 << 30;
@@ -89,12 +95,12 @@
                     const int ns = (t.w + e->TW - 1) / e->TW;
                     const int nr = (t.h + ro - 1) / ro, sh = (t.h + nr - 1) / nr;
                     njobs += (long long)ns * nr;
-                    rows = std::max(rows, sh);
+                    for (int sy = 0; sy < t.h; sy += sh) rows = std::max(rows, les::march_rows(t.y + sy, std::min(sh, t.h - sy), frs[i].y, R, sched));
                     useful = std::max(useful, (t.w + ns - 1) / ns);
                 }
                 if (njobs == 0) continue;
                 const long long wgs = (njobs + e->NJ - 1) / e->NJ;
-                const double ticks = (double)((rows + 4 * R + e->BY - 1) / e->BY + 3);
+                const double ticks = (double)((rows + e->BY - 1) / e->BY + 3);
                 const double cost = (double)((wgs + ncu - 1) / ncu) * ticks * (1.0 + 1e-3 * (double)wgs / ncu) + (ro == (1 << 30) ? 0.0 : 1e-6);
                 if (cost < best) { best = cost; m = e; max_rows = ro; }
             }
@@ -163,7 +169,7 @@
         hipLaunchKernelGGL(les::les_naive_raw_kernel, dim3(rp->n, rp->chunks), dim3(256), 0, stream, c->geom, strip_view(c, mode), rp->calls, d_planes, rp->raw);
         mv.vol = rp->raw; mv.raw_off = rp->off;
     }
-    hipLaunchKernelGGL(m->fn, dim3(ngroups), dim3(m->NT), 0, stream, c->geom, mv, d_mjobs, d_planes, d_out, ngroups, check);
+    hipLaunchKernelGGL(m->fn, dim3(ngroups), dim3(m->NT), 0, stream, c->geom, mv, d_mjobs, d_planes, d_out, ngroups, check, march_sched());
     HIPCHECK(hipGetLastError());
     return LES_HIP_OK;
 }
@@ -220,7 +226,7 @@
                            rp.raw, (unsigned*)nullptr, -INFINITY);
     }
     HIPCHECK(hipGetLastError());
-    if (ngroups > 0) hipLaunchKernelGGL(m->fn, dim3(ngroups), dim3(m->NT), 0, stream, c->geom, mv, d_mjobs, d_planes, d_out, ngroups, check);
+    if (ngroups > 0) hipLaunchKernelGGL(m->fn, dim3(ngroups), dim3(m->NT), 0, stream, c->geom, mv, d_mjobs, d_planes, d_out, ngroups, check, march_sched());
     HIPCHECK(hipGetLastError());
     if (quad && nsjobs > 0) {
         hipLaunchKernelGGL(les::les_mask_jobs_kernel, dim3((nsjobs + 255) / 256), dim3(256), 0, stream, d_sjobs, d_rjobs, (const unsigned*)d_flags, nsjobs);
diff --git a/localexpstereo_amd/csrc/les_hip_march_tables.inc b/localexpstereo_amd/csrc/les_hip_march_tables.inc
--- a/localexpstereo_amd/csrc/les_hip_march_tables.inc
+++ b/localexpstereo_amd/csrc/les_hip_march_tables.inc
@@ -51,7 +51,7 @@
     return def;
 }
 
-typedef void (*MarchKernel)(les::Geom, les::MarchView, const les::Job*, const float4*, float*, int, int);
+typedef void (*MarchKernel)(les::Geom, les::MarchView, const les::Job*, const float4*, float*, int, int, int);
 struct MarchEntry { int R; int TW; int NJ; int NT; int BY; MarchKernel fn; };
 #define LES_MARCH_ENTRY(R_, WGC_, NJ_, BY_) \
     { R_, les::MarchCfg<R_, WGC_, NJ_, BY_>::TW, NJ_, les::MarchCfg<R_, WGC_, NJ_, BY_>::NT, BY_, les::les_march_kernel<R_, WGC_, NJ_, BY_> }
diff --git a/localexpstereo_amd/csrc/les_hip_vdisp.inc b/localexpstereo_amd/csrc/les_hip_vdisp.inc
--- a/localexpstereo_amd/csrc/les_hip_vdisp.inc
+++ b/localexpstereo_amd/csrc/les_hip_vdisp.inc
@@ -13,7 +13,7 @@
     launch_naive_raw(c, mode, rp.calls, rp.n, rp.chunks, d_planes, rp.raw, stream);
     les::MarchView mv = c->v[mode].mv;
     mv.vol = rp.raw; mv.raw_off = rp.off;
-    hipLaunchKernelGGL(m->fn, dim3(ngroups), dim3(m->NT), 0, stream, c->geom, mv, d_mjobs, d_planes, d_out, ngroups, check);
+    hipLaunchKernelGGL(m->fn, dim3(ngroups), dim3(m->NT), 0, stream, c->geom, mv, d_mjobs, d_planes, d_out, ngroups, check, march_sched());
     HIPCHECK(hipGetLastError());
     return LES_HIP_OK;
 }
diff --git a/localexpstereo_amd/csrc/les_march.h b/localexpstereo_amd/csrc/les_march.h
--- a/localexpstereo_amd/csrc/les_march.h
+++ b/localexpstereo_amd/csrc/les_march.h
@@ -9,6 +9,11 @@
 #define LES_STATS_POLICY ""
 #define LES_LAB_ROLE_ON(bit) true
 #define LES_LAB_ABLATE(bit) false
+#endif
+#if defined(LES_SIM)
+#define LES_MARCH_OPAQUE(v_) ((void)0)
+#else
+#define LES_MARCH_OPAQUE(v_) asm volatile("" : "+v"(v_))
 #endif
 #ifndef LES_TICK_BEGIN
 #define LES_TICK_BEGIN() ((void)0)
@@ -53,9 +58,16 @@
 #define LES_TILED_MIN_SLOPE 0.125f
 #endif
 
+#ifndef LES_MARCH_CA_R10
+#define LES_MARCH_CA_R10 1
+#endif
+__host__ __device__ constexpr int march_ca(int R) { return R == 10 ? LES_MARCH_CA_R10 : 0; }
+
 template <int R, int WGC, int NJ, int BY>
 struct MarchCfg {
     static constexpr int KS = 2 * R + 1;
+    static constexpr int CA = march_ca(R);
+    static_assert(CA >= 0 && CA < BY, "role C keeps at least one row of its block");
     static constexpr int RS = 3 * BY;
     static constexpr int TW = WGC - 4 * R;
     static constexpr int HWV = WGC / 64;
@@ -117,10 +129,11 @@
     }
 }
 
-template <int BY, int PCOLS>
+template <int BY, int PCOLS, bool LOCAL = false>
 __device__ __forceinline__ void march_prefix_pair(int4 (*TA)[PCOLS], int4 (*TB)[PCOLS], int ci0, int lane)
 {
     constexpr int SEGL = 8;
+    if constexpr (LOCAL) LES_MARCH_OPAQUE(lane);
     const int row = 2 * (lane >> 4) + (lane & 1), seg = (lane & 15) >> 1;
     const bool act = row < BY;
     const int c0 = ci0 + seg * SEGL;
@@ -209,6 +222,48 @@
 #else
     return __float_as_int(r.c.x);
 #endif
+}
+#if defined(LES_SIM) || defined(LES_MARCH_STATS_PLAIN)
+typedef MarchStatDesc MarchStatPlainDesc;
+__device__ inline MarchStatPlainDesc march_stats_plain_desc(const float* base, uint32_t bytes) { return march_stats_desc(base, bytes); }
+__device__ inline void march_stats_load_plain(MarchStatRow& r, const MarchStatPlainDesc& d, uint32_t voff, uint32_t soff) { march_stats_load(r, d, voff, soff); }
+#else
+typedef BufRsrc MarchStatPlainDesc;
+__device__ __forceinline__ MarchStatPlainDesc march_stats_plain_desc(const float* base, uint32_t bytes) { return make_buf(base, bytes); }
+__device__ __forceinline__ void march_stats_load_plain(MarchStatRow& r, MarchStatPlainDesc d, uint32_t voff, uint32_t soff)
+{
+    r.a = __builtin_bit_cast(mstat4, __builtin_amdgcn_raw_buffer_load_b128(d, (int)voff, (int)soff, 0));
+    r.b = __builtin_bit_cast(mstat4, __builtin_amdgcn_raw_buffer_load_b128(d, (int)(voff + 16u), (int)soff, 0));
+#if LES_MARCH_STAT_WORDS == 9
+    r.c = __builtin_bit_cast(float, __builtin_amdgcn_raw_buffer_load_b32(d, (int)(voff + 32u), (int)soff, 0));
+#else
+    r.c = __builtin_bit_cast(mstat4, __builtin_amdgcn_raw_buffer_load_b128(d, (int)(voff + 32u), (int)soff, 0));
+#endif
+}
+#endif
+
+__device__ __forceinline__ void march_c_row(const int4& pp, const int4& pm, const int4& px, const MarchStatRow& st, float rny, float kap_x, float up_x,
+                                            float kmu, int4* dst)
+{
+    const int s = pp.x - pm.x + px.x;
+    const mstat4 q0 = st.a, q1 = st.b;
+    const int M0 = __float_as_int(q1.z), M1 = __float_as_int(q1.w), M2 = march_stat_m2(st);
+    const long long s8 = (long long)(s << kMarchSL);
+    const float d0 = (float)((pp.y - pm.y) + px.y + (int)(((long long)M0 * s8 + (1ll << 31)) >> 32));
+    const float d1 = (float)((pp.z - pm.z) + px.z + (int)(((long long)M1 * s8 + (1ll << 31)) >> 32));
+    const float d2 = (float)((pp.w - pm.w) + px.w + (int)(((long long)M2 * s8 + (1ll << 31)) >> 32));
+    const float ka = kap_x * rny;
+    const float a0 = fmaf(q0.z, d2, fmaf(q0.y, d1, q0.x * d0)) * ka;
+    const float a1 = fmaf(q1.x, d2, fmaf(q0.w, d1, q0.y * d0)) * ka;
+    const float a2 = fmaf(q1.y, d2, fmaf(q1.x, d1, q0.z * d0)) * ka;
+    const float mp = (float)s * (up_x * rny);
+#if LES_MARCH_STAT_WORDS == 9
+    const float bb = fmaf(kmu, fmaf(a2, (float)M2, fmaf(a1, (float)M1, a0 * (float)M0)), mp);
+#else
+    (void)kmu;
+    const float bb = fmaf(-a2, st.c.w, fmaf(-a1, st.c.z, fmaf(-a0, st.c.y, mp)));
+#endif
+    lds_store4(dst, cvt_rpi_i32(a0), cvt_rpi_i32(a1), cvt_rpi_i32(a2), cvt_rpi_i32(bb));
 }
 
 __device__ __forceinline__ bool march_label_surely_valid(const Geom& g, float4 pl, int x0, int x1, int y0, int y1)
@@ -242,10 +297,20 @@
     return s0 >= 0 && s1 < g.D && (unsigned long long)(s1 - s0 + 1) * HW < (1ull << 28);
 }
 
+__host__ __device__ inline int march_lead_in(int ty0, int cy0, int R, int sched)
+{
+    const int t0 = cy0 - (ty0 - 2 * R);
+    return (sched & 1) && t0 > 0 ? t0 : 0;
+}
+__host__ __device__ inline int march_rows(int ty0, int th, int cy0, int R, int sched)
+{
+    return th > 0 ? th + 4 * R - march_lead_in(ty0, cy0, R, sched) : 0;
+}
+
 template <int R, int WGC, int NJ, int BY>
 __global__ void __launch_bounds__(3 * WGC * NJ)
 les_march_kernel(Geom g, MarchView view, const Job* __restrict__ jobs, const float4* __restrict__ planes,
-                 float* __restrict__ out, int ngroups, int check)
+                 float* __restrict__ out, int ngroups, int check, int sched)
 {
     using Cfg = MarchCfg<R, WGC, NJ, BY>;
     constexpr int KS = Cfg::KS, RS = Cfg::RS, NT = Cfg::NT, HWV = Cfg::HWV, PCOLS = Cfg::PCOLS;
@@ -269,12 +334,17 @@
     const int slot = wave / (3 * HWV), role = kRoleOf[LES_MARCH_ROLE_ORDER][(wave % (3 * HWV)) / HWV], half = wave % HWV;
     const int ci0 = half * 64, ci = ci0 + lane;
     const Job job = jobs[grp * NJ + slot];
-    int th_max = 0;
-#pragma unroll
-    for (int s = 0; s < NJ; s++) th_max = max(th_max, jobs[grp * NJ + s].th);
-    const int nblk = (th_max + 4 * R + BY - 1) / BY;
+    int rows_max = 0;
+#pragma unroll
+    for (int s = 0; s < NJ; s++) {
+        const Job js = jobs[grp * NJ + s];
+        rows_max = max(rows_max, march_rows(js.ty0, js.th, js.cy0, R, sched));
+    }
+    const int nblk = (rows_max + BY - 1) / BY;
     const int nticks = nblk + 3;
-    const int Ttot = job.th > 0 ? job.th + 4 * R : 0;
+    const int t0 = march_lead_in(job.ty0, job.cy0, R, sched);
+    const int y_org = job.ty0 - 2 * R + t0;
+    const int Ttot = march_rows(job.ty0, job.th, job.cy0, R, sched);
     const float4 plane = planes[job.plane_idx];
     const int cy1m = max(job.cy1 - 1, job.cy0);
 
@@ -299,6 +369,13 @@
     const bool cross = cM >= 0 && (cP >> 6) != (cM >> 6);
     const int pcX = cross ? Cfg::pcol((cP >> 6) * 64 - 1) : 0;
     const int pcS = Cfg::pcol(ci);
+    const bool s1_col = col_in && ci >= R && ci < WGC - R;
+    const float rnx = s1_col ? s_rtab[nx] : 0.0f;
+    const float kap_x = view.kapS * rnx;
+    const float up_x = view.upS * rnx;
+    const uint32_t sxS = (uint32_t)sx * (uint32_t)(4 * kMarchStatWords);
+    const uint32_t rowS = (uint32_t)g.W * (uint32_t)(4 * kMarchStatWords);
+    const bool lend_job = Cfg::CA > 0 && (sched & 2) != 0 && (view.raw_off || (plane.x == 0.0f && plane.y == 0.0f));
 
     if (role == 0 && LES_LAB_ROLE_ON(1)) {
         const uint32_t HWu = (uint32_t)g.H * (uint32_t)g.W;
@@ -321,15 +398,19 @@
         const bool tame = !fronto && !view.raw_off && march_plane_short_gather(g, plane, job, R, &slice_lo);
         const uint32_t W8 = ((uint32_t)g.W + 7u) >> 3;
         const uint32_t trowB = W8 * (uint32_t)g.D * 32u;
-        const int trow_lo = max(job.ty0 - 2 * R, job.cy0);
-        const int trow_hi = min(job.ty0 - 2 * R + (nblk + 2) * BY, job.cy1);
+        const int trow_lo = max(y_org, job.cy0);
+        const int trow_hi = min(y_org + (nblk + 2) * BY, job.cy1);
         const unsigned long long tspanB = (unsigned long long)max(trow_hi - trow_lo, 1) * (unsigned long long)trowB;
         const bool tiled = tame && view.vol_t && fabsf(plane.x) >= (NJ == 1 ? LES_TILED_MIN_SLOPE_WIDE : LES_TILED_MIN_SLOPE) && tspanB < 0xfffffff0ull &&
                            (unsigned long long)W8 * (unsigned long long)g.D * 32ull < (1ull << 31);
         const float spj = !col_in ? 0.0f : (inv_job ? 0.0f : view.sp);
         const float pmj = !col_in ? __int_as_float(kMarchMagicBits) : (inv_job ? fmaf(g.th_col, view.sp, view.pmagic) : view.pmagic);
-        auto march_a = [&](auto kind_tag) __attribute__((always_inline)) {
+        auto march_a = [&](auto kind_tag, auto lend_tag) __attribute__((always_inline)) {
         constexpr int KIND = decltype(kind_tag)::value;
+        constexpr int CA = decltype(lend_tag)::value ? Cfg::CA : 0;
+        static_assert(CA == 0 || KIND == 0 || KIND == 1 || KIND == 3, "only the marches with the paired prefix pass have the registers for a lent row");
+        constexpr int CAN = CA > 0 ? CA : 1;
+        const MarchStatPlainDesc ds_lent = march_stats_plain_desc(view.mstats, (uint32_t)g.H * rowS);
         GatherPrep gp[BY];
         float v0[BY], v1[BY];
         float f1r[BY];
@@ -353,7 +434,7 @@
         const BufRsrc rs_v1 = make_buf(view.vol + (size_t)i1s, imgB);
         auto prep = [&](int b) __attribute__((always_inline)) {
             const int t = b * BY + lane;
-            const int gy = job.ty0 - 2 * R + t;
+            const int gy = y_org + t;
             const int sy = min(max(gy, job.cy0), cy1m);
             nx_rowB = (int)((uint32_t)sy * rowB);
             rowbits_nx = ballot_low(t < Ttot && gy >= job.cy0 && gy < job.cy1, BY);
@@ -407,6 +488,32 @@
                 constexpr int BASE = decltype(utag)::value * BY;
                 const int k = k0 + decltype(utag)::value;
                 if (k < nticks) {
+                    const bool lent = CA > 0 && k >= 1 && k <= nblk;
+                    MarchStatRow lst[CAN];
+                    int4 lpp[CAN], lpm[CAN], lpx[CAN];
+                    float lrny[CAN];
+                    if constexpr (CA > 0) {
+                        if (lent) {
+                            const int4 (*T1p)[PCOLS] = s_T1[(k - 1) & 1][slot];
+                            int cl = ci;
+                            LES_MARCH_OPAQUE(cl);
+                            const int cPl = min(cl + R, WGC - 1), cMl = cl - R - 1;
+                            const int pcPl = Cfg::pcol(cPl), pcMl = cMl >= 0 ? Cfg::pcol(cMl) : 0;
+                            const int pcXl = (cMl >= 0 && (cPl >> 6) != (cMl >> 6)) ? Cfg::pcol((cPl >> 6) * 64 - 1) : 0;
+                            uint32_t sx4l = sx4;
+                            LES_MARCH_OPAQUE(sx4l);
+                            const uint32_t sxSl = sx4l * (uint32_t)kMarchStatWords;
+#pragma unroll
+                            for (int j = 0; j < CA; j++) {
+                                const int t = (k - 1) * BY + (BY - CA + j);
+                                const int gy1 = y_org - R + t;
+                                const bool on = gy1 >= job.cy0 && gy1 < job.cy1 && gy1 >= job.ty0 - R && t < Ttot;
+                                lrny[j] = on ? s_rtab[window_count(gy1, R, job.cy0, job.cy1)] : 0.0f;
+                                march_stats_load_plain(lst[j], ds_lent, sxSl, (uint32_t)min(max(gy1, job.cy0), cy1m) * rowS);
+                                lpp[j] = T1p[BY - CA + j][pcPl]; lpm[j] = T1p[BY - CA + j][pcMl]; lpx[j] = T1p[BY - CA + j][pcXl];
+                            }
+                        }
+                    }
                     if (k < nblk) {
                         int4 (*T)[PCOLS] = s_T1[k & 1][slot];
                         prep(k + 1);
@@ -447,11 +554,22 @@
                         rowbits = rowbits_nx;
                         LES_TICK_MARK();
                     }
+                    if constexpr (CA > 0) {
+                        if (lent) {
+                            int4 (*T2w)[PCOLS] = s_T2[(decltype(utag)::value + UN - 1) % UN][slot];
+                            float rnxl = rnx;
+                            LES_MARCH_OPAQUE(rnxl);
+                            const float kap_xl = view.kapS * rnxl, up_xl = view.upS * rnxl;
+#pragma unroll
+                            for (int j = 0; j < CA; j++)
+                                march_c_row(lpp[j], lpm[j], lpx[j], lst[j], lrny[j], kap_xl, up_xl, view.kmu, &T2w[BY - CA + j][pcS]);
+                        }
+                    }
                     {
                         int4 (*TB)[PCOLS] = s_T2[(decltype(utag)::value + UN - 2 % UN) % UN][slot];
                         const bool da = k < nblk, db = !(NJ > 1 && KIND == 2) && k >= 2 && k < nblk + 2;
                         constexpr bool kPair = KIND != 2 && KIND != 4 && KIND != 5;
-                        if (kPair && da && db) march_prefix_pair<BY, PCOLS>(s_T1[k & 1][slot], TB, ci0, lane);
+                        if (kPair && da && db) march_prefix_pair<BY, PCOLS, (CA > 0)>(s_T1[k & 1][slot], TB, ci0, lane);
                         else {
                             if (da) { wave_sync(); march_prefix_tile<BY, PCOLS>(s_T1[k & 1][slot], ci0, lane); }
                             if (db) march_prefix_tile<BY, PCOLS>(TB, ci0, lane);
@@ -463,24 +581,26 @@
         }
         LES_TICK_END(0);
         };
-        if (view.raw_off) march_a(std::integral_constant<int, 3>{});
-        else if (fronto && f1s == 0.0f) march_a(std::integral_constant<int, 0>{});
-        else if (fronto) march_a(std::integral_constant<int, 1>{});
-        else if (tiled) march_a(std::integral_constant<int, 5>{});
-        else if (tame) march_a(std::integral_constant<int, 4>{});
-        else march_a(std::integral_constant<int, 2>{});
+        constexpr std::false_type kOwn{};
+        auto march_a_lending = [&](auto kind_tag) __attribute__((always_inline)) {
+            if constexpr (Cfg::CA > 0) { if (lend_job) { march_a(kind_tag, std::true_type{}); return; } }
+            march_a(kind_tag, kOwn);
+        };
+        if (view.raw_off) march_a_lending(std::integral_constant<int, 3>{});
+        else if (fronto && f1s == 0.0f) march_a_lending(std::integral_constant<int, 0>{});
+        else if (fronto) march_a_lending(std::integral_constant<int, 1>{});
+        else if (tiled) march_a(std::integral_constant<int, 5>{}, kOwn);
+        else if (tame) march_a(std::integral_constant<int, 4>{}, kOwn);
+        else march_a(std::integral_constant<int, 2>{}, kOwn);
     } else if (role == 1 && LES_LAB_ROLE_ON(2)) {
-        const bool s1_col = col_in && ci >= R && ci < WGC - R;
         int slice_lo_unused = 0;
         const bool general_plane = !view.raw_off && !(plane.x == 0.0f && plane.y == 0.0f) && !march_plane_short_gather(g, plane, job, R, &slice_lo_unused);
-        const float kap_x = s1_col ? view.kapS * s_rtab[nx] : 0.0f;
-        const float up_x = s1_col ? view.upS * s_rtab[nx] : 0.0f;
-        const uint32_t sxS = (uint32_t)sx * (uint32_t)(4 * kMarchStatWords);
-        const uint32_t rowS = (uint32_t)g.W * (uint32_t)(4 * kMarchStatWords);
         const MarchStatDesc ds_stats = march_stats_desc(view.mstats, (uint32_t)g.H * rowS);
-        MarchStatRow st[BY];
-#pragma unroll
-        for (int i = 0; i < BY; i++) {
+        auto march_c = [&](auto nc_tag) __attribute__((always_inline)) {
+        constexpr int NC = decltype(nc_tag)::value;
+        MarchStatRow st[NC];
+#pragma unroll
+        for (int i = 0; i < NC; i++) {
             st[i].a = st[i].b = mstat4{0.0f, 0.0f, 0.0f, 0.0f};
 #if LES_MARCH_STAT_WORDS == 9
             st[i].c = 0.0f;
@@ -488,13 +608,13 @@
             st[i].c = mstat4{0.0f, 0.0f, 0.0f, 0.0f};
 #endif
         }
-        float rny[BY];
+        float rny[NC];
         int nx_srow = 0;
         float nx_rny = 0.0f;
         auto prep = [&](int b) __attribute__((always_inline)) {
             const int t = b * BY + lane;
-            const int gy1 = job.ty0 - 3 * R + t;
-            const bool on = gy1 >= job.cy0 && gy1 < job.cy1 && t >= 2 * R && t < Ttot;
+            const int gy1 = y_org - R + t;
+            const bool on = gy1 >= job.cy0 && gy1 < job.cy1 && gy1 >= job.ty0 - R && t < Ttot;
             nx_rny = on ? s_rtab[window_count(gy1, R, job.cy0, job.cy1)] : 0.0f;
             nx_srow = (int)((uint32_t)min(max(gy1, job.cy0), cy1m) * rowS);
         };
@@ -507,21 +627,21 @@
             march_stats_load(st[i], ds_stats, sxS, soff);
         };
         prep(0);
-        static_for<BY>([&](auto itag) { issue_row(itag); });
+        static_for<NC>([&](auto itag) { issue_row(itag); });
         LES_TICK_BEGIN();
         for (int k = 0; k < nticks; k++) {
             if (k >= 1 && k <= nblk) {
                 const int b = k - 1;
                 const int4 (*T1)[PCOLS] = s_T1[b & 1][slot];
                 int4 (*T2)[PCOLS] = s_T2[b % 3][slot];
-                constexpr int GC = 2, NS = (BY + GC - 1) / GC;
+                constexpr int GC = 2, NS = (NC + GC - 1) / GC;
                 prep(k);
                 int4 pp[2][GC], pm[2][GC], px[2][GC];
                 auto lds_stage = [&](auto stag) __attribute__((always_inline)) {
                     constexpr int S = decltype(stag)::value;
 #pragma unroll
                     for (int j = 0; j < GC; j++)
-                        if (S * GC + j < BY) {
+                        if (S * GC + j < NC) {
                             if (LES_LAB_ABLATE(2)) { pp[S & 1][j] = int4{lane, k, 2, 3}; pm[S & 1][j] = int4{3, 2, k, lane}; px[S & 1][j] = int4{0, 0, 0, 0}; }
                             else { pp[S & 1][j] = T1[S * GC + j][pcP]; pm[S & 1][j] = T1[S * GC + j][pcM]; px[S & 1][j] = T1[S * GC + j][pcX]; }
                         }
@@ -530,33 +650,16 @@
                 static_for<NS>([&](auto gtag) {
                     constexpr int S = decltype(gtag)::value, CB = S & 1;
                     constexpr int LO = S * GC;
-                    constexpr int N = (BY - LO) < GC ? (BY - LO) : GC;
+                    constexpr int N = (NC - LO) < GC ? (NC - LO) : GC;
                     if constexpr (S + 1 < NS) lds_stage(std::integral_constant<int, S + 1>{});
                     LES_MARCH_SCHED_FENCE();
                     static_assert(GC == 2, "vmcnt bookkeeping below is written for stages of two rows");
-                    if constexpr (N == 2) march_stats_wait<3 * (BY - 2)>(st[LO], st[LO + 1]);
-                    else march_stats_wait<3 * (BY - 1)>(st[LO]);
+                    if constexpr (N == 2) march_stats_wait<3 * (NC - 2)>(st[LO], st[LO + 1]);
+                    else march_stats_wait<3 * (NC - 1)>(st[LO]);
                     static_for<N>([&](auto jtag) {
                         constexpr int j = decltype(jtag)::value;
                         constexpr int i = LO + j;
-                        const int s = pp[CB][j].x - pm[CB][j].x + px[CB][j].x;
-                        const mstat4 q0 = st[i].a, q1 = st[i].b;
-                        const int M0 = __float_as_int(q1.z), M1 = __float_as_int(q1.w), M2 = march_stat_m2(st[i]);
-                        const long long s8 = (long long)(s << kMarchSL);
-                        const float d0 = (float)((pp[CB][j].y - pm[CB][j].y) + px[CB][j].y + (int)(((long long)M0 * s8 + (1ll << 31)) >> 32));
-                        const float d1 = (float)((pp[CB][j].z - pm[CB][j].z) + px[CB][j].z + (int)(((long long)M1 * s8 + (1ll << 31)) >> 32));
-                        const float d2 = (float)((pp[CB][j].w - pm[CB][j].w) + px[CB][j].w + (int)(((long long)M2 * s8 + (1ll << 31)) >> 32));
-                        const float ka = kap_x * rny[i];
-                        const float a0 = fmaf(q0.z, d2, fmaf(q0.y, d1, q0.x * d0)) * ka;
-                        const float a1 = fmaf(q1.x, d2, fmaf(q0.w, d1, q0.y * d0)) * ka;
-                        const float a2 = fmaf(q1.y, d2, fmaf(q1.x, d1, q0.z * d0)) * ka;
-                        const float mp = (float)s * (up_x * rny[i]);
-#if LES_MARCH_STAT_WORDS == 9
-                        const float bb = fmaf(view.kmu, fmaf(a2, (float)M2, fmaf(a1, (float)M1, a0 * (float)M0)), mp);
-#else
-                        const float bb = fmaf(-a2, st[i].c.w, fmaf(-a1, st[i].c.z, fmaf(-a0, st[i].c.y, mp)));
-#endif
-                        lds_store4(&T2[i][pcS], cvt_rpi_i32(a0), cvt_rpi_i32(a1), cvt_rpi_i32(a2), cvt_rpi_i32(bb));
+                        march_c_row(pp[CB][j], pm[CB][j], px[CB][j], st[i], rny[i], kap_x, up_x, view.kmu, &T2[i][pcS]);
                     });
                     LES_MARCH_SCHED_FENCE();
                     static_for<N>([&](auto jtag) { issue_row(std::integral_constant<int, LO + decltype(jtag)::value>{}); });
@@ -567,6 +670,11 @@
             LES_TICK_BARRIER();
         }
         LES_TICK_END(1);
+        };
+        if constexpr (Cfg::CA > 0) {
+            if (lend_job) march_c(std::integral_constant<int, BY - Cfg::CA>{});
+            else march_c(std::integral_constant<int, BY>{});
+        } else march_c(std::integral_constant<int, BY>{});
     } else if (role == 2 && LES_LAB_ROLE_ON(4)) {
         const bool out_col = ci >= 2 * R && ci < 2 * R + job.tw && job.th > 0;
         const uint32_t oc4 = (uint32_t)max(ci - 2 * R, 0) * 4u;
@@ -583,12 +691,13 @@
         float nx_rny = 0.0f;
         const BufRsrc rs_out = make_buf(out + job.out_off, 0xfffffffcu);
         const uint32_t ostrideB = (uint32_t)job.out_stride * 4u;
+        const int orow0 = 4 * R - t0;
         auto prep = [&](int b) __attribute__((always_inline)) {
             const int t = b * BY + lane;
-            const int gy2 = job.ty0 - 4 * R + t;
+            const int gy2 = y_org - 2 * R + t;
             nx_rny = s_rtab[window_count(gy2, R, job.cy0, job.cy1)];
             nx_grow = (int)((uint32_t)min(max(gy2, job.cy0), cy1m) * rowB);
-            okbits = ballot_low(t >= 4 * R && t < Ttot, BY);
+            okbits = ballot_low(t >= orow0 && t < Ttot, BY);
         };
         auto issue_row = [&](auto itag) __attribute__((always_inline)) {
             constexpr int i = decltype(itag)::value;
@@ -642,7 +751,7 @@
                                     const float acc = fmaf(f2, cvt_f32_sbyte<2>(gi), fmaf(f1, cvt_f32_sbyte<1>(gi), fmaf(f0, cvt_f32_sbyte<0>(gi), f3 * 255.0f)));
                                     float q = fmaf(acc * c_lane, rny2[i], view.poff);
                                     if constexpr (CHECK) {
-                                        const int gy2 = job.ty0 + t - 4 * R;
+                                        const int gy2 = job.ty0 + (t - orow0);
                                         const float ds = ((vl_xa + (float)gy2 * plane.y) + vl_c) + vl_zv;
                                         const float dp = ds + vl_a5, dm = ds - vl_a5;
                                         const float d1 = dp + vl_b5, d2 = dp - vl_b5, d3 = dm + vl_b5, d4 = dm - vl_b5;
@@ -650,7 +759,7 @@
                                         if (!(mn >= g.mind && mx <= g.maxd)) q = LES_COST_INVALID;
                                     }
                                     if (!(LES_LAB_ABLATE(128) && q != 12345.0f))
-                                    buf_store<float>(rs_out, oc4, (uint32_t)(t - 4 * R) * ostrideB, q);
+                                    buf_store<float>(rs_out, oc4, (uint32_t)(t - orow0) * ostrideB, q);
                                 }
                             });
                             LES_MARCH_SCHED_FENCE();
```

New measurement: 146,100. -13.4%, worse.
